# yesint/molar

Hardware: AMD Instinct MI355X
Metric: frames/sec + Matom-pairs/sec, 1M-atom PBC neighbor search + RMSD fit (higher is better)
Workload: dtype f32; 1 GPU; 1M-atom synthetic triclinic box A, per frame: PBC neighbour search rc=1.2 nm (ordered pair list in HBM) + Kabsch RMSD fit/COM/gyration of a 100k-atom selection; natoms=1000000, selection_atoms=100000, frames_per_gpu=1451, parallelism=frames sharded over 1 rank(s), no data-path collective, streams_per_gpu=2, measure_overlapped_with_search=True

## Files before the change

include/molar_hip.h:

```cpp
#ifndef MOLAR_HIP_H
#define MOLAR_HIP_H

#include <stddef.h>
#include <stdint.h>

#ifdef __cplusplus
extern "C" {
#endif

enum {
    MOLAR_HIP_OK = 0,
    MOLAR_HIP_ERR_SIZES = 1,
    MOLAR_HIP_ERR_ZERO_MASS = 2,
    MOLAR_HIP_ERR_SVD = 3,
    MOLAR_HIP_ERR_NO_PBC = 4,
    MOLAR_HIP_ERR_ZERO_LENGTH_VECTOR = 5,
    MOLAR_HIP_ERR_INVERSE_FAILED = 6,
    MOLAR_HIP_ERR_LIPID_TAIL_TOO_SHORT = 7,
    MOLAR_HIP_ERR_LIPID_NORMALS_COUNT = 8,
    MOLAR_HIP_ERR_LIPID_BOND_ORDER_COUNT = 9,
    MOLAR_HIP_ERR_ANGLE_TOO_SMALL = 10,
    MOLAR_HIP_ERR_INVALID_ARGUMENT = 50,
    MOLAR_HIP_ERR_TOO_LARGE = 51,
    MOLAR_HIP_ERR_NO_SEARCH = 52,
// ... 35 lines not shown
int molar_hip_box_from_vectors_angles(float a, float b, float c, float alpha, float beta, float gamma,
                                      molar_hip_box *out);
void molar_hip_box_shortest_vector(const molar_hip_box *box, const float v[3], uint8_t pbc, float out[3]);
void molar_hip_box_lab_extents(const molar_hip_box *box, float out[3]);
void molar_hip_box_extents(const molar_hip_box *box, float out[3]);
void molar_hip_box_to_box_coords(const molar_hip_box *box, const float v[3], float out[3]);
void molar_hip_box_to_lab_coords(const molar_hip_box *box, const float v[3], float out[3]);
int molar_hip_box_is_inside(const molar_hip_box *box, const float p[3]);
void molar_hip_box_wrap_point(const molar_hip_box *box, const float p[3], float out[3]);


enum {
    MOLAR_HIP_SEARCH_SINGLE = 0,
    MOLAR_HIP_SEARCH_DOUBLE = 1,
    MOLAR_HIP_SEARCH_WITHIN = 2,
    MOLAR_HIP_SEARCH_DOUBLE_VDW = 3
};

typedef struct {
    int32_t kind;
    float cutoff;
    const float *xyz1;
    size_t natoms1;
    const uint64_t *idx1;
    size_t n1;
    const float *xyz2;
    size_t natoms2;
    const uint64_t *idx2;
    size_t n2;
    const float *vdw1;
    const float *vdw2;
    int32_t ids_local;
    const float *box9;
    uint8_t pbc;
    const float *lower3;
    const float *upper3;
} molar_hip_search_desc;

int molar_hip_search_count(molar_hip_ctx *ctx, const molar_hip_search_desc *desc, uint64_t *out_count);
int molar_hip_search_fill(molar_hip_ctx *ctx, uint32_t *pairs, float *dist);
int molar_hip_search_fill_usize(molar_hip_ctx *ctx, uint64_t *i, uint64_t *j, float *dist);
int molar_hip_search_fill_ids(molar_hip_ctx *ctx, uint64_t *ids);
int molar_hip_within_count(molar_hip_ctx *ctx, const molar_hip_search_desc *desc, uint64_t *out_count);
int molar_hip_within_fill(molar_hip_ctx *ctx, uint64_t *ids);
int molar_hip_within_hold(molar_hip_ctx *ctx, int on);
int molar_hip_search_connectivity(molar_hip_ctx *ctx, const molar_hip_search_desc *desc, uint64_t *out_rows, uint64_t *out_entries);
int molar_hip_search_connectivity_fill(molar_hip_ctx *ctx, uint64_t *offsets, uint64_t *neigh);
int molar_hip_unwrap_connectivity(molar_hip_ctx *ctx, float *xyz, size_t natoms, const uint64_t *idx, size_t n,
                                  const float *box9, float cutoff, uint8_t pbc_dims, uint64_t *group_offsets,
                                  uint64_t *group_ids, size_t *ngroups);
int molar_hip_search_grid_dims(molar_hip_ctx *ctx, uint64_t dims[3]);
int molar_hip_search_cell_kernels(molar_hip_ctx *ctx, int32_t *lanes, uint64_t occupied_cells[2]);
int molar_hip_search_slot_counts(molar_hip_ctx *ctx, uint64_t *slots, uint64_t *consecutive_slots);
int molar_hip_search_fill_device(molar_hip_ctx *ctx, const uint32_t **d_pairs, const float **d_dist);
int molar_hip_search_resident(molar_hip_ctx *ctx, const molar_hip_search_desc *desc, uint64_t *out_count,
                              const uint32_t **d_pairs, const float **d_dist);
int molar_hip_search_resident_planes(molar_hip_ctx *ctx, int want_dist);
int molar_hip_search_resident_begin(molar_hip_ctx *ctx, const molar_hip_search_desc *desc, int32_t *ticket);
int molar_hip_search_resident_end(molar_hip_ctx *ctx, int32_t ticket, uint64_t *out_count, const uint32_t **d_pairs,
                                  const float **d_dist);
int molar_hip_search_histogram(molar_hip_ctx *ctx, const molar_hip_search_desc *desc, float hmin,
                               float hmax, size_t nbins, uint64_t *bins, uint64_t *out_count);
int molar_hip_search_histogram_frames(molar_hip_ctx *ctx, const molar_hip_search_desc *desc, size_t nframes, size_t xyz1_stride,
                                      size_t xyz2_stride, const float *boxes9, float hmin, float hmax, size_t nbins,
                                      uint64_t *bins);
int molar_hip_histogram_edges(float hmin, float hmax, size_t nbins, float *edges);

typedef struct {
    const uint32_t *group1;
    size_t ngroups1;
    const uint32_t *group2;
    size_t ngroups2;
} molar_hip_contact_groups;

int molar_hip_search_contacts(molar_hip_ctx *ctx, const molar_hip_search_desc *desc, const molar_hip_contact_groups *groups ,
                              uint64_t *deg1, uint64_t *deg2, uint64_t *map, uint64_t *out_count);
int molar_hip_search_contacts_frames(molar_hip_ctx *ctx, const molar_hip_search_desc *desc, const molar_hip_contact_groups *groups,
                                     size_t nframes, size_t xyz1_stride, size_t xyz2_stride, const float *boxes9,
                                     uint64_t *deg1, uint64_t *deg2, uint64_t *map, uint32_t *occupancy);

int molar_hip_search_clusters(molar_hip_ctx *ctx, const molar_hip_search_desc *desc, const molar_hip_contact_groups *groups ,
                              uint32_t *comp_of, uint32_t *sizes, uint64_t *offsets, uint32_t *members, uint32_t *out_ncomponents);
int molar_hip_search_clusters_frames(molar_hip_ctx *ctx, const molar_hip_search_desc *desc, const molar_hip_contact_groups *groups,
                                     size_t nframes, size_t xyz1_stride, const float *boxes9, uint32_t *ncomponents, uint32_t *largest,
                                     uint64_t *size_hist, uint32_t *comp_of_frames);
int molar_hip_search_clusters_counters(molar_hip_ctx *ctx, int32_t enable, uint64_t *out4);

enum {
    MOLAR_HIP_HBOND_DHA_MIN = 0,
    MOLAR_HIP_HBOND_HDA_MAX = 1
};
int molar_hip_hbonds_count(molar_hip_ctx *ctx, const molar_hip_search_desc *desc, const uint64_t *h_offsets, const uint64_t *h_idx,
                           size_t nh, int32_t angle_kind, double angle_deg, double max_ha, uint64_t *out_count);
int molar_hip_hbonds_fill(molar_hip_ctx *ctx, uint32_t *triples, double *dist_da, double *dist_ha, double *angle_deg);
int molar_hip_hbonds_counts(molar_hip_ctx *ctx, const molar_hip_search_desc *desc, const uint64_t *h_offsets, const uint64_t *h_idx,
                            size_t nh, int32_t angle_kind, double angle_deg, double max_ha, const molar_hip_contact_groups *groups,
                            uint64_t *don_count, uint64_t *acc_count, uint64_t *map, uint64_t *out_count);
int molar_hip_hbonds_frames(molar_hip_ctx *ctx, const molar_hip_search_desc *desc, const uint64_t *h_offsets, const uint64_t *h_idx,
                            size_t nh, int32_t angle_kind, double angle_deg, double max_ha, size_t nframes, size_t xyz_stride,
                            const float *boxes9, const molar_hip_contact_groups *groups, uint64_t *per_frame, uint64_t *don_count,
                            uint64_t *acc_count, uint64_t *map, uint64_t *out_total, uint64_t *out_unique);
int molar_hip_hbonds_frames_fill(molar_hip_ctx *ctx, uint64_t *frame_offsets, uint32_t *triples, double *dist_da, double *dist_ha,
                                 double *angle_deg, uint32_t *bond_of_entry, uint32_t *table, uint32_t *occupancy);

int molar_hip_lifetimes_plan(size_t nframes, size_t nrows, size_t ngroups, int want_cont, size_t *workspace_bytes,
                             uint32_t *words_per_row);
// ... 480 lines not shown
```

molar_amd/_lib.py:

```python
from __future__ import annotations

import ctypes as C
import os

HERE = os.path.dirname(os.path.abspath(__file__))
DEFAULT_LIB = os.path.join(HERE, "libmolar_hip.so")

_lib = None


class MolarHipError(RuntimeError):

    def __init__(self, code: int, msg: str):
        super().__init__(f"[molar_hip status {code}] {msg}")
        self.code = code


class Box(C.Structure):
    _fields_ = [("m", C.c_float * 9), ("inv", C.c_float * 9), ("nshift", C.c_int32), ("shifts", C.c_float * 78)]


class SearchDesc(C.Structure):
    _fields_ = [
        ("kind", C.c_int32), ("cutoff", C.c_float),
# ... 49 lines not shown
        ("masses", C.c_void_p), ("ntails", C.c_size_t), ("tail_idx", C.c_void_p), ("tail_offsets", C.c_void_p),
        ("tail_lipid", C.c_void_p), ("tail_bonds", C.c_void_p),
        ("cutoff", C.c_float), ("order_type", C.c_int32), ("max_smooth_iter", C.c_int32), ("unwrap", C.c_int32),
        ("use_global_normal", C.c_int32), ("global_normal", C.c_float * 3),
    ]


MEMBRANE_ARRAYS = ("head", "mid", "tail", "patch_offsets", "patch_ids", "initial_normals", "valid", "smoothed_head", "normals",
                   "quad_coefs", "mean_curv", "gauss_curv", "princ_curvs", "princ_dirs", "area", "nvert", "neib_ids",
                   "voro_vertexes", "fitted_patch_points", "order")


class MembraneView(C.Structure):
    _fields_ = ([("nlipids", C.c_size_t), ("patch_entries", C.c_size_t), ("npairs", C.c_size_t)]
                + [(k, C.c_void_p) for k in MEMBRANE_ARRAYS] + [("norder", C.c_size_t)])


class MembraneOut(C.Structure):
    _fields_ = [(k, C.c_void_p) for k in MEMBRANE_ARRAYS]


_P, _SZ, _F, _I, _U8 = C.c_void_p, C.c_size_t, C.c_float, C.c_int, C.c_uint8
SYMBOLS = {
    "molar_hip_create": (C.c_void_p, [_I]),
    "molar_hip_destroy": (None, [_P]),
    "molar_hip_last_error": (C.c_char_p, []),
    "molar_hip_version": (C.c_char_p, []),
    "molar_hip_device_count": (_I, []),
    "molar_hip_set_stream": (_I, [_P, _P]),
    "molar_hip_synchronize": (_I, [_P]),
    "molar_hip_profile_enable": (_I, [_P, _I]),
    "molar_hip_profile_read": (_I, [_P, _P, _P]),
    "molar_hip_box_from_matrix": (_I, [_P, _P]),
    "molar_hip_box_from_vectors_angles": (_I, [_F, _F, _F, _F, _F, _F, _P]),
    "molar_hip_box_shortest_vector": (None, [_P, _P, _U8, _P]),
    "molar_hip_copy_bandwidth": (_I, [_P, _SZ, _I, _P]),
    "molar_hip_write_bandwidth": (_I, [_P, _SZ, _I, _P]),
    "molar_hip_box_lab_extents": (None, [_P, _P]),
    "molar_hip_box_extents": (None, [_P, _P]),
    "molar_hip_box_to_box_coords": (None, [_P, _P, _P]),
    "molar_hip_box_to_lab_coords": (None, [_P, _P, _P]),
    "molar_hip_box_is_inside": (_I, [_P, _P]),
    "molar_hip_box_wrap_point": (None, [_P, _P, _P]),
    "molar_hip_search_count": (_I, [_P, _P, _P]),
    "molar_hip_search_fill": (_I, [_P, _P, _P]),
    "molar_hip_search_fill_usize": (_I, [_P, _P, _P, _P]),
    "molar_hip_search_fill_ids": (_I, [_P, _P]),
    "molar_hip_within_count": (_I, [_P, _P, _P]),
    "molar_hip_within_fill": (_I, [_P, _P]),
    "molar_hip_within_hold": (_I, [_P, _I]),
    "molar_hip_search_grid_dims": (_I, [_P, _P]),
    "molar_hip_search_cell_kernels": (_I, [_P, _P, _P]),
    "molar_hip_search_slot_counts": (_I, [_P, _P, _P]),
    "molar_hip_search_count_f64": (_I, [_P, _P, _P]),
    "molar_hip_search_fill_f64": (_I, [_P, _P, _P, _P]),
    "molar_hip_search_fill_ids_f64": (_I, [_P, _P]),
    "molar_hip_search_grid_dims_f64": (_I, [_P, _P]),
    "molar_hip_search_histogram_f64": (_I, [_P, _P, C.c_double, C.c_double, _SZ, _P, _P]),
    "molar_hip_search_histogram_frames_f64": (_I, [_P, _P, _SZ, _SZ, _SZ, _P, C.c_double, C.c_double, _SZ, _P]),
    "molar_hip_histogram_edges_f64": (_I, [C.c_double, C.c_double, _SZ, _P]),
    "molar_hip_within_count_f64": (_I, [_P, _P, _P]),
    "molar_hip_within_fill_f64": (_I, [_P, _P]),
    "molar_hip_search_connectivity_f64": (_I, [_P, _P, _P, _P]),
    "molar_hip_unwrap_connectivity_f64": (_I, [_P, _P, _SZ, _P, _SZ, _P, C.c_double, _U8, _P, _P, _P]),
    "molar_hip_search_resident": (_I, [_P, _P, _P, _P, _P]),
    "molar_hip_search_fill_device": (_I, [_P, _P, _P]),
    "molar_hip_search_resident_planes": (_I, [_P, _I]),
    "molar_hip_search_resident_begin": (_I, [_P, _P, _P]),
    "molar_hip_search_resident_end": (_I, [_P, C.c_int32, _P, _P, _P]),
    "molar_hip_search_histogram": (_I, [_P, _P, _F, _F, _SZ, _P, _P]),
    "molar_hip_search_histogram_frames": (_I, [_P, _P, _SZ, _SZ, _SZ, _P, _F, _F, _SZ, _P]),
    "molar_hip_histogram_edges": (_I, [_F, _F, _SZ, _P]),
    "molar_hip_search_contacts": (_I, [_P, _P, _P, _P, _P, _P, _P]),
    "molar_hip_search_contacts_frames": (_I, [_P, _P, _P, _SZ, _SZ, _SZ, _P, _P, _P, _P, _P]),
    "molar_hip_search_clusters": (_I, [_P, _P, _P, _P, _P, _P, _P, _P]),
    "molar_hip_search_clusters_frames": (_I, [_P, _P, _P, _SZ, _SZ, _P, _P, _P, _P, _P]),
    "molar_hip_search_clusters_counters": (_I, [_P, C.c_int32, _P]),
    "molar_hip_min_max": (_I, [_P, _P, _SZ, _P, _SZ, _P, _P]),
    "molar_hip_center_of_geometry": (_I, [_P, _P, _SZ, _P, _SZ, _P]),
    "molar_hip_center_of_mass": (_I, [_P, _P, _SZ, _P, _SZ, _P, _P]),
    "molar_hip_center_of_geometry_pbc": (_I, [_P, _P, _SZ, _P, _SZ, _P, _U8, _P]),
    "molar_hip_center_of_mass_pbc": (_I, [_P, _P, _SZ, _P, _SZ, _P, _P, _U8, _P]),
    "molar_hip_gyration": (_I, [_P, _P, _SZ, _P, _SZ, _P, _P, _P]),
    "molar_hip_inertia": (_I, [_P, _P, _SZ, _P, _SZ, _P, _P, _P, _P, _P]),
    "molar_hip_rmsd": (_I, [_P, _P, _SZ, _P, _SZ, _P, _SZ, _P, _SZ, _P]),
    "molar_hip_rmsd_mw": (_I, [_P, _P, _SZ, _P, _SZ, _P, _P, _SZ, _P, _SZ, _P]),
    "molar_hip_fit_transform": (_I, [_P, _P, _SZ, _P, _SZ, _P, _P, _SZ, _P, _SZ, _P, _I, _P, _P]),
    "molar_hip_xtc_histogram": (_I, [_P, _P, _SZ, _SZ, _P, _SZ, _F, _U8, _F, _F, _SZ, _P, _I]),
    "molar_hip_xtc_histogram_double": (_I, [_P, _P, _SZ, _SZ, _P, _SZ, _P, _SZ, _F, _U8, _F, _F, _SZ, _P, _I]),
    "molar_hip_fit_stream_create": (_I, [_P, _SZ, _P, _SZ, _P, _P, _SZ, _P, _I, _P]),
    "molar_hip_fit_stream_begin": (_I, [_P, _P, _I, _P]),
    "molar_hip_fit_stream_end": (_I, [_P, C.c_int32, _P, _P, _P, _P, _P]),
    "molar_hip_fit_stream_destroy": (None, [_P]),
    "molar_hip_center_of_geometry_f64": (_I, [_P, _P, _SZ, _P, _SZ, _P]),
    "molar_hip_center_of_mass_f64": (_I, [_P, _P, _SZ, _P, _SZ, _P, _P]),
    "molar_hip_gyration_f64": (_I, [_P, _P, _SZ, _P, _SZ, _P, _P]),
    "molar_hip_rmsd_f64": (_I, [_P, _P, _SZ, _P, _SZ, _P, _SZ, _P, _SZ, _P]),
    "molar_hip_rmsd_mw_f64": (_I, [_P, _P, _SZ, _P, _SZ, _P, _P, _SZ, _P, _SZ, _P]),
    "molar_hip_fit_transform_f64": (_I, [_P, _P, _SZ, _P, _SZ, _P, _P, _SZ, _P, _SZ, _P, _I, _P, _P]),
    "molar_hip_apply_transform_f64": (_I, [_P, _P, _SZ, _P, _SZ, _P, _P]),
    "molar_hip_fit_rmsd_batch_f64": (_I, [_P, _P, _SZ, _SZ, _P, _SZ, _P, _P, _SZ, _P, _I, _P, _P, _P, _P, _P]),
    "molar_hip_center_of_geometry_pbc_f64": (_I, [_P, _P, _SZ, _P, _SZ, _P, _U8, _P]),
    "molar_hip_center_of_mass_pbc_f64": (_I, [_P, _P, _SZ, _P, _SZ, _P, _P, _U8, _P]),
    "molar_hip_gyration_pbc_f64": (_I, [_P, _P, _SZ, _P, _SZ, _P, _P, _P]),
    "molar_hip_unwrap_simple_f64": (_I, [_P, _P, _SZ, _P, _SZ, _P, _U8]),
    "molar_hip_inertia_pbc_f64": (_I, [_P, _P, _SZ, _P, _SZ, _P, _P, _P, _P, _P]),
# ... 140 lines not shown
```

molar_amd/api.py:

```python
from __future__ import annotations

import collections
import ctypes as C

import numpy as np

from . import _lib
from ._lib import (MEMBRANE_ARRAYS, Box, ContactGroups, MembraneDesc, MembraneOut, MembraneView, MolarHipError, SearchDesc, SearchDescF64,
                   check)

PBC_FULL = 7
PBC_NONE = 0

SEARCH_SINGLE, SEARCH_DOUBLE, SEARCH_WITHIN, SEARCH_DOUBLE_VDW = 0, 1, 2, 3

ERR_NO_SEARCH = 52
LIFETIME_OUTPUTS = ("inter", "cont", "run_hist", "events", "longest", "present")


def _is_torch(x) -> bool:
    return type(x).__module__.startswith("torch")


def _addr(x):
# ... 202 lines not shown
        d = SearchDesc()
        d.kind = kind
        d.cutoff = float(cutoff) if cutoff is not None else 0.0
        keep = []
        for name, arr in (("xyz1", xyz1), ("idx1", idx1), ("xyz2", xyz2), ("idx2", idx2), ("vdw1", vdw1),
                          ("vdw2", vdw2)):
            a, k = _addr(arr)
            setattr(d, name, a)
            keep.append(k)
        d.natoms1 = 0 if xyz1 is None else xyz1.shape[0] if xyz1.ndim == 2 else xyz1.shape[0] // 3
        d.natoms2 = 0 if xyz2 is None else xyz2.shape[0] if xyz2.ndim == 2 else xyz2.shape[0] // 3
        d.n1 = 0 if idx1 is None else idx1.shape[0]
        d.n2 = 0 if idx2 is None else idx2.shape[0]
        d.ids_local = 1 if ids_local else 0
        if box is not None:
            b9 = box.colmajor9() if isinstance(box, PeriodicBox) else np.ascontiguousarray(
                np.asarray(box, np.float32).reshape(3, 3).T).reshape(9)
            keep.append(b9)
            d.box9 = b9.ctypes.data
        d.pbc = pbc_mask(pbc)
        if lower is not None:
            lo = np.ascontiguousarray(lower, np.float32); up = np.ascontiguousarray(upper, np.float32)
            keep += [lo, up]
            d.lower3 = lo.ctypes.data
            d.upper3 = up.ctypes.data
        return d, keep

    def search_count(self, kind, cutoff, xyz1, idx1=None, xyz2=None, idx2=None, box=None, pbc=0, vdw1=None,
                     vdw2=None, ids_local=False, lower=None, upper=None) -> int:
        d, keep = self._search_desc(kind, cutoff, xyz1, idx1, xyz2, idx2, box, pbc, vdw1, vdw2, ids_local, lower, upper)
        cnt = C.c_uint64(0)
        check(self.lib.molar_hip_search_count(self.ctx, C.byref(d), C.byref(cnt)))
        self._keep = keep
        return int(cnt.value)

    def make_search_desc(self, kind, cutoff, xyz1, **kw):
        return self._search_desc(kind, cutoff, xyz1, **kw)

    def search_resident_desc(self, desc):
        cnt = C.c_uint64(0); p = C.c_void_p(); dd = C.c_void_p()
        check(self.lib.molar_hip_search_resident(self.ctx, C.byref(desc), C.byref(cnt), C.byref(p), C.byref(dd)))
        return int(cnt.value), p.value, dd.value

    def search_cell_kernels(self):
        lanes = C.c_int32(-1)
        occ = (C.c_uint64 * 2)()
        check(self.lib.molar_hip_search_cell_kernels(self.ctx, C.byref(lanes), occ))
        return int(lanes.value), (int(occ[0]), int(occ[1]))

    def search_slot_counts(self):
        slots, rows = C.c_uint64(0), C.c_uint64(0)
        check(self.lib.molar_hip_search_slot_counts(self.ctx, C.byref(slots), C.byref(rows)))
        return int(slots.value), int(rows.value)

    def search_resident_planes(self, want_dist=True):
        check(self.lib.molar_hip_search_resident_planes(self.ctx, 1 if want_dist else 0))

    def search_resident_begin(self, desc):
        t = C.c_int32(-1)
        check(self.lib.molar_hip_search_resident_begin(self.ctx, C.byref(desc), C.byref(t)))
        return int(t.value)

    def search_resident_end(self, ticket):
        cnt = C.c_uint64(0); p = C.c_void_p(); dd = C.c_void_p()
        check(self.lib.molar_hip_search_resident_end(self.ctx, C.c_int32(ticket), C.byref(cnt), C.byref(p), C.byref(dd)))
        return int(cnt.value), p.value, dd.value

    def search_resident(self, kind, cutoff, xyz1, idx1=None, xyz2=None, idx2=None, box=None, pbc=0, vdw1=None,
                        vdw2=None, ids_local=False, lower=None, upper=None):
        d, keep = self._search_desc(kind, cutoff, xyz1, idx1, xyz2, idx2, box, pbc, vdw1, vdw2, ids_local, lower, upper)
        cnt = C.c_uint64(0); p = C.c_void_p(); dd = C.c_void_p()
        check(self.lib.molar_hip_search_resident(self.ctx, C.byref(d), C.byref(cnt), C.byref(p), C.byref(dd)))
        self._keep = keep
        return int(cnt.value), p.value, dd.value

    def search_fill(self, count):
        pairs = np.empty((count, 2), np.uint32)
        dist = np.empty(count, np.float32)
        check(self.lib.molar_hip_search_fill(self.ctx, pairs.ctypes.data, dist.ctypes.data))
        return pairs, dist

    def search_fill_usize(self, count):
        i = np.empty(count, np.uint64); j = np.empty(count, np.uint64); d = np.empty(count, np.float32)
        check(self.lib.molar_hip_search_fill_usize(self.ctx, i.ctypes.data, j.ctypes.data, d.ctypes.data))
        return i, j, d

    def within_set(self, cutoff, xyz1, idx1=None, xyz2=None, idx2=None, box=None, pbc=0, ids_local=False, lower=None,
                   upper=None, device_out=None):
        d, keep = self._search_desc(SEARCH_WITHIN, cutoff, xyz1, idx1, xyz2, idx2, box, pbc, None, None, ids_local, lower, upper)
        cnt = C.c_uint64(0)
        check(self.lib.molar_hip_within_count(self.ctx, C.byref(d), C.byref(cnt)))
        self._keep = keep
        n = int(cnt.value)
        if device_out is not None:
            out = device_out(n)
            if n:
                check(self.lib.molar_hip_within_fill(self.ctx, out.data_ptr()))
            return out
        ids = np.empty(n, np.uint64)
        if n:
            check(self.lib.molar_hip_within_fill(self.ctx, ids.ctypes.data))
        return ids

    def search_connectivity(self, cutoff, xyz, idx=None, box=None, pbc=0, ids_local=True):
        d, keep = self._search_desc(SEARCH_SINGLE, cutoff, xyz, idx, None, None, box, pbc, None, None, ids_local, None, None)
        rows, ent = C.c_uint64(0), C.c_uint64(0)
# ... 2913 lines not shown
```

molar_amd/csrc/api.hip:

```cpp
#include "boxmath.hpp"
#include <algorithm>

#include "common.hpp"
#include "hoststream.hpp"
#include <cstdlib>

using namespace mh;

typedef float v4f_copy __attribute__((ext_vector_type(4)));
__global__ __launch_bounds__(256) void k_copy_f4(const float4 *__restrict__ src, float4 *__restrict__ dst, size_t n) {
    for (size_t i = (size_t)blockIdx.x * 256u + threadIdx.x; i < n; i += (size_t)gridDim.x * 256u) dst[i] = src[i];
}
template <bool NT>
__global__ __launch_bounds__(256) void k_copy_f4x4(const v4f_copy *__restrict__ src, v4f_copy *__restrict__ dst, size_t n) {
    for (size_t i = (size_t)blockIdx.x * 1024u + threadIdx.x; i < n; i += (size_t)gridDim.x * 1024u) {
        v4f_copy v0, v1, v2, v3;
        if (NT) {
            v0 = __builtin_nontemporal_load(src + i);
            v1 = __builtin_nontemporal_load(src + i + 256);
            v2 = __builtin_nontemporal_load(src + i + 512);
            v3 = __builtin_nontemporal_load(src + i + 768);
            __builtin_nontemporal_store(v0, dst + i);
            __builtin_nontemporal_store(v1, dst + i + 256);
            __builtin_nontemporal_store(v2, dst + i + 512);
// ... 77 lines not shown

const char *molar_hip_last_error(void) { return last_error().c_str(); }

const char *molar_hip_version(void) { return "molar_hip 0.2 (gfx950)"; }

int molar_hip_device_count(void) {
    int n = 0;
    if (hipGetDeviceCount(&n) != hipSuccess) {
        (void)hipGetLastError();
        return 0;
    }
    return n;
}

molar_hip_ctx *molar_hip_create(int device) {
    int n = 0;
    hipError_t e = hipGetDeviceCount(&n);
    if (e != hipSuccess || n == 0) {
        (void)hipGetLastError();
        fail(MOLAR_HIP_ERR_HIP, "molar_hip_create: no HIP device visible (%s)",
             e == hipSuccess ? "device count is 0" : hipGetErrorString(e));
        return nullptr;
    }
    if (device < 0 || device >= n) {
        fail(MOLAR_HIP_ERR_INVALID_ARGUMENT, "molar_hip_create: device %d out of range [0,%d)", device, n);
        return nullptr;
    }
    if ((e = hipSetDevice(device)) != hipSuccess) {
        fail(MOLAR_HIP_ERR_HIP, "hipSetDevice(%d): %s", device, hipGetErrorString(e));
        return nullptr;
    }
    hipDeviceProp_t prop;
    if ((e = hipGetDeviceProperties(&prop, device)) != hipSuccess) {
        fail(MOLAR_HIP_ERR_HIP, "hipGetDeviceProperties: %s", hipGetErrorString(e));
        return nullptr;
    }
    auto *c = new molar_hip_ctx();
    c->device = device;
    c->num_cus = prop.multiProcessorCount > 0 ? prop.multiProcessorCount : 256;
    if ((e = hipStreamCreateWithFlags(&c->stream, hipStreamNonBlocking)) != hipSuccess) {
        fail(MOLAR_HIP_ERR_HIP, "hipStreamCreate: %s", hipGetErrorString(e));
        delete c;
        return nullptr;
    }
    c->own_stream = true;
#ifdef MOLAR_HIP_AB_KNOBS
    c->env_no_side = std::getenv("MOLAR_HIP_NO_SIDE_STREAM") != nullptr;
    c->env_no_mfma = std::getenv("MOLAR_HIP_NO_MFMA_COUNT") != nullptr;
    c->env_no_mfma_wrapped = std::getenv("MOLAR_HIP_NO_MFMA_WRAPPED") != nullptr;
    c->env_no_tile_sum = std::getenv("MOLAR_HIP_NO_TILE_SUM") != nullptr;
    c->env_host_grid_wait = std::getenv("MOLAR_HIP_HOST_GRID_WAIT") != nullptr;
    c->env_no_bin_tile = std::getenv("MOLAR_HIP_NO_BIN_TILE") != nullptr;
#endif
#ifdef MOLAR_HIP_DEBUG_KNOBS
    if (const char *dbg = std::getenv("MOLAR_HIP_DEBUG_SKIP")) c->env_debug_skip = (uint32_t)std::atoi(dbg);
    if (const char *dbg = std::getenv("MOLAR_HIP_DEBUG_LAUNCH")) c->env_debug_launch = (uint32_t)std::atoi(dbg);
#endif
    if (ensure_pinned(c, 1 << 16) || alloc_search_sizes(c)) {
        if (c->h_pinned) (void)hipHostFree(c->h_pinned);
        (void)hipStreamDestroy(c->stream);
        delete c;
        return nullptr;
    }
    return c;
}

void molar_hip_destroy(molar_hip_ctx *c) {
    if (!c) return;
    (void)hipSetDevice(c->device);
    (void)hipStreamSynchronize(c->stream);
    if (c->side_stream) (void)hipStreamSynchronize(c->side_stream);
    if (c->aux) molar_hip_destroy(c->aux);
    mh::contacts_release(c);
    if (c->hb_pin) (void)hipHostFree(c->hb_pin);
    for (auto e : c->hb_pin_ev)
        if (e) (void)hipEventDestroy(e);
    for (auto &s : c->spans) {
        (void)hipEventDestroy(s.a);
        (void)hipEventDestroy(s.b);
    }
    for (auto e : c->event_pool) (void)hipEventDestroy(e);
    if (c->h_pinned) (void)hipHostFree(c->h_pinned);
    mh::ring_release(c);
    mh::search64_release(c);
    mh::sasa_release(c);
    mh::rmsd_matrix_release(c);
    mh::fluct_release(c);
    mh::msd_release(c);
    mh::density_release(c);
    mh::intcoord_release(c);
    mh::tcf_release(c);
    mh::sfactor_release(c);
    mh::mindist_release(c);
    mh::hbonds_release(c);
    mh::lifetimes_release(c);
    mh::within_release(c);
    mh::connectivity_release(c);
    if (c->h_sizes) (void)hipHostFree(c->h_sizes);
    for (auto &t : c->tickets)
        if (t.done) (void)hipEventDestroy(t.done);
    if (c->grid_done) (void)hipEventDestroy(c->grid_done);
    for (auto e : c->gen_free)
        if (e) (void)hipEventDestroy(e);
    if (c->side_stream) (void)hipStreamDestroy(c->side_stream);
    if (c->own_stream) (void)hipStreamDestroy(c->stream);
    delete c;
// ... 127 lines not shown
```

molar_amd/csrc/common.hpp:

```cpp
#pragma once

#include <hip/hip_runtime.h>

#include <cstdarg>
#include <cstddef>
#include <cstdint>
#include <cstdio>
#include <cstring>
#include <string>
#include <utility>
#include <vector>

#include "../../include/molar_hip.h"

namespace mh {


inline std::string &last_error() {
    static thread_local std::string e;
    return e;
}

inline int fail(int code, const char *fmt, ...) {
    char buf[512];
// ... 151 lines not shown
struct molar_hip_sfactor_state;
struct molar_hip_mindist_state;
struct molar_hip_hbonds_state;
struct molar_hip_lifetimes_state;
struct molar_hip_within_state;
struct molar_hip_connectivity_state;
struct molar_hip_contacts_state;

#ifndef MH_HIST_BATCH
#define MH_HIST_BATCH 16
#endif

struct molar_hip_ctx {
    int device = 0;
    hipStream_t stream = nullptr;
    bool own_stream = false;
    int num_cus = 256;

    void *h_pinned = nullptr;
    size_t h_pinned_cap = 0;
    molar_hip_search64_state *s64 = nullptr;
    molar_hip_sasa_state *sasa = nullptr;
    molar_hip_rmsd_matrix_state *rmsdm = nullptr;
    molar_hip_fluct_state *fluct = nullptr;
    molar_hip_msd_state *msd = nullptr;
    molar_hip_density_state *density = nullptr;
    molar_hip_intcoord_state *intcoord = nullptr;
    molar_hip_tcf_state *tcf = nullptr;
    molar_hip_sfactor_state *sfactor = nullptr;
    molar_hip_mindist_state *mindist = nullptr;
    molar_hip_hbonds_state *hbonds = nullptr;
    molar_hip_lifetimes_state *lifetimes = nullptr;
    molar_hip_within_state *within = nullptr;
    molar_hip_connectivity_state *conn = nullptr;
    molar_hip_contacts_state *contacts = nullptr;
    void *ring[8] = {nullptr, nullptr, nullptr, nullptr, nullptr, nullptr, nullptr, nullptr};
    hipEvent_t ring_ev[8] = {nullptr, nullptr, nullptr, nullptr, nullptr, nullptr, nullptr, nullptr};

    bool have_search = false;
    mh::SearchShape cur;
    uint64_t total = 0;
    mh::GridSet set_store[2][2];
    molar_hip_ctx() { cur.set = set_store[0]; }
    hipStream_t side_stream = nullptr;
    hipEvent_t grid_done = nullptr;
    bool env_no_side = false;
    bool env_no_mfma = false;
    bool env_no_mfma_wrapped = false;
    bool env_host_grid_wait = false;
    bool env_no_tile_sum = false;
    uint32_t env_debug_skip = 0;
    uint32_t env_debug_launch = 0, dbg_launches = 0;
    hipEvent_t gen_free[2] = {nullptr, nullptr};
    bool env_no_bin_tile = false;
    int hist_gen = 0;
    mh::DevBuf scan_tmp_side;
    mh::DevBuf params;
    mh::DevBuf task_desc;
    mh::DevBuf task_nb;
    mh::DevBuf slot_desc;
    mh::DevBuf slot_cnt;
    mh::DevBuf slot_base;
    mh::DevBuf tile_sum;
    bool params_fresh = false;
    unsigned long long params_fresh_cap = 0;
    mh::DevBuf scan_tmp;
    mh::DevBuf sort_tmp, sort_tmp_side;
    mh::DevBuf scan_state;
    mh::DevBuf fplan_tiles;
    mh::DevBuf slot_stat;
    bool slot_stat_valid = false;
    bool plan_live = false;
    mh::DevBuf out_pairs_set[2];
    mh::DevBuf out_dist_set[2];
    mh::DevBuf &out_pairs = out_pairs_set[0];
    mh::DevBuf &out_dist = out_dist_set[0];
    struct Ticket {
        bool pending = false, degenerate = false;
        unsigned long long cap0 = 0, maskcap0 = 0, serial = 0, launched = 0, ntasks = 0;
        int kind = -1;
        unsigned long long occ_key = 0;
        hipEvent_t done = nullptr;
        molar_hip_search_desc desc{};
    } tickets[2];
    int next_ticket = 0;
    bool resident_no_dist = false;
    unsigned long long search_serial = 0;
    unsigned long long trim_real = 0, trim_ntasks = 0;
    int trim_kind = -1;
    static constexpr int SIZES_SYNC = 2, SIZES_ENTRIES = 3;
    mh::SearchSizes *h_sizes = nullptr, *d_sizes = nullptr;
    unsigned long long occ_key = 0;
    uint32_t occ_cells[2] = {0, 0};
    bool occ_valid = false;
    mh::DevBuf out_ids;
    mh::DevBuf wide_i, wide_j;
    mh::DevBuf hist;
    mh::DevBuf dbg;
    mh::DevBuf hist_queue;
    mh::DevBuf slot_desc_rest;
    unsigned long long hist_frames = 0;
    mh::GridSet hb_sets[2][MH_HIST_BATCH][2];
    bool hb_zeroed[2][MH_HIST_BATCH][2] = {};
    uint32_t hb_zeroed_cells[2][MH_HIST_BATCH][2] = {};
    mh::DevBuf hb_lean[2], hb_rest[2];
    mh::DevBuf hb_blocks[2];
    void *hb_pin = nullptr;
    hipEvent_t hb_pin_ev[4] = {nullptr, nullptr, nullptr, nullptr};
    bool hb_pin_used[4] = {false, false, false, false};
    unsigned hb_pin_next = 0;
    mh::DevBuf hist_edges;
    float edges_min = 0.f, edges_max = 0.f;
    size_t edges_nbins = 0;
    bool within_hold = false;
    mh::HeldGrid held;
    mh::DevBuf task_mu;
    mh::DevBuf task_moff;
    mh::DevBuf maskbuf;
    uint64_t mask_units = 0;

    molar_hip_ctx *aux = nullptr;
    mh::DevBuf xh_win[2], xh_bins;

    bool profiling = false;
    bool profile_frames = false;
    struct Span { int cls; hipEvent_t a, b; };
    std::vector<Span> spans;
    std::vector<hipEvent_t> event_pool;

    mh::DevBuf fit_redo;
    mh::DevBuf m_xyz1, m_xyz2, m_idx1, m_idx2, m_mass1, m_mass2, m_partials, m_results, m_out;
};

namespace mh {

void search64_release(molar_hip_ctx *c);
void sasa_release(molar_hip_ctx *c);
void rmsd_matrix_release(molar_hip_ctx *c);
void fluct_release(molar_hip_ctx *c);
void msd_release(molar_hip_ctx *c);
void density_release(molar_hip_ctx *c);
void intcoord_release(molar_hip_ctx *c);
void tcf_release(molar_hip_ctx *c);
void sfactor_release(molar_hip_ctx *c);
void mindist_release(molar_hip_ctx *c);
void hbonds_release(molar_hip_ctx *c);
void lifetimes_release(molar_hip_ctx *c);
void within_release(molar_hip_ctx *c);
void connectivity_release(molar_hip_ctx *c);
void contacts_release(molar_hip_ctx *c);


template <class State>
State &state_of(State *&slot) {
    if (!slot) slot = new State;
    return *slot;
}

template <class State>
void release_state(State *&slot) {
    delete slot;
    slot = nullptr;
}

struct HbondsBlockView {
    const uint64_t *frame_offsets;
    size_t nframes;
    const uint32_t *bond_of_entry;
    size_t rows, entries;
    uint64_t serial;
};
// ... 88 lines not shown
```

molar_amd/csrc/pair_kernels.hpp:

```cpp
#pragma once

#include "boxmath.hpp"
#include "common.hpp"

namespace mh {
namespace pairk {

enum { MODE_COUNT = 0, MODE_FILL = 1, MODE_HIST = 2 };

#ifndef MH_COUNT_WPE
#define MH_COUNT_WPE 6
#endif
#ifndef MH_FILL_WPE
#define MH_FILL_WPE 8
#endif
#ifndef MH_WPB
#define MH_WPB 1
#endif
constexpr int waves_per_block(int mode) { return mode == MODE_HIST ? 4 : MH_WPB; }
constexpr int KREG = 8;
constexpr int FIFO_CAP = 128;
constexpr int LIVE_GROUPS = KREG;
constexpr uint32_t SLOT_LIVE = 0x400u;
#ifndef MOLAR_HIP_NO_WIDE_FLUSH
// ... 25 lines not shown
__device__ __forceinline__ void gstore_u32(uint32_t *p, size_t i, uint32_t v) {
    ((__attribute__((address_space(1))) uint32_t *)p)[i] = v;
}
__device__ __forceinline__ float uniform_f32(float v) { return __uint_as_float(__builtin_amdgcn_readfirstlane(__float_as_uint(v))); }
__device__ __forceinline__ float4 lload4(const float4 *p, uint32_t i) {
    const v4f_t v = ((const __attribute__((address_space(3))) v4f_t *)p)[i];
    return make_float4(v.x, v.y, v.z, v.w);
}

struct SearchParams {
    const float4 *sa;
    const float4 *sb;
    const uint32_t *csa;
    const uint32_t *csb;
    const float *vdwa;
    const float *vdwb;
    const float4 *aabb_b;
    const float4 *perm_b;
    const float4 *chunk_aabb_b;
    const uint4 *h16_b;
    const float4 *cell_org_b;
    uint32_t mfma_count;
    const struct TaskDesc *task_desc;
    uint32_t *maskbuf;
    const unsigned long long *task_moff;
    unsigned long long mask_cap_units;
    unsigned long long out_cap;
    uint32_t dx, dy, dz;
    uint32_t pbc;
    uint32_t use_box;
    uint32_t nblocks;
    uint32_t wrap_kind;
    uint32_t prune_wrapped;
    float prune_limit2;
    uint32_t approx_wrapped;
    float band_lo, band_hi;
    uint32_t hist_nbins;
    float hist_min, hist_max;
    unsigned long long *hist_bins;
    unsigned long long *hist_total;
    const float *hist_edges;
    float hist_scale;
    uint32_t hist_lean;
    const uint32_t *hist_nslots;
#ifdef MOLAR_HIP_DEBUG_KNOBS
    uint32_t debug_skip;
    unsigned long long *dbg;
#endif
    float cutoff2;
    uint64_t ntasks;
    molar_hip_box box;
    alignas(16) float shifts4[96];
    uint32_t hist_big;
};

struct TaskDesc {
    uint32_t a0, n1, b0, n2, cb, flags, pad0, pad1;
};

struct SlotDesc {
    uint32_t a0, n1, b0, n2;
    uint32_t cb, flags, i0, frame;
    unsigned long long moff, pad1;
};
static_assert(sizeof(SlotDesc) == 48, "SlotDesc is read with three 16-byte loads");

struct Task {
    uint32_t a0, n1, b0, n2;
    uint32_t rps;
    uint32_t cb;
    uint32_t ca;
    uint32_t wrap_b;
    uint32_t wrap;
    bool tri;
    bool valid;
};

struct SlotTask : Task {
    bool live = false;
    uint32_t lrow = 0;
};

__device__ __forceinline__ uint32_t slot_row(const SlotTask &T, uint32_t i0, uint32_t lane) { return T.live ? T.lrow : i0 + lane; }

template <int KIND, bool UNIFORM>
__device__ __forceinline__ Task decode_task(const SearchParams &P, uint64_t t) {
    Task T;
    T.valid = false;
    T.tri = false;
    T.a0 = T.b0 = T.n1 = T.n2 = 0;
    T.cb = 0;
    T.ca = 0;
    T.wrap_b = 0;
    T.rps = 64u;
    T.wrap = 0;
    uint32_t half = 0;
    uint64_t e = t;
    if (KIND != MOLAR_HIP_SEARCH_SINGLE) {
        half = (uint32_t)(t & 1ull);
        e = t >> 1;
    }
    const uint32_t m = (uint32_t)(e % 14ull);
    const uint64_t cidx = e / 14ull;
    const uint32_t z = (uint32_t)(cidx % P.dz);
    const uint64_t r = cidx / P.dz;
    const uint32_t y = (uint32_t)(r % P.dy);
    const uint32_t x = (uint32_t)(r / P.dy);
    const uint32_t dims[3] = {P.dx, P.dy, P.dz};
    uint32_t c[2][3] = {{x + MASKS[m][0], y + MASKS[m][1], z + MASKS[m][2]},
                        {x + MASKS[m][3], y + MASKS[m][4], z + MASKS[m][5]}};
    uint32_t wrap = 0, wrap_c2 = 0;
    for (int i = 0; i < 2; ++i)
        for (int d = 0; d < 3; ++d)
            if (c[i][d] == dims[d]) {
                if ((P.pbc >> d) & 1u) {
                    c[i][d] = 0;
                    wrap |= 1u << d;
                    if (i == 1) wrap_c2 |= 1u << d;
                } else {
                    return T;
                }
            }
    const uint32_t i1 = c[0][0] + c[0][1] * P.dx + c[0][2] * P.dx * P.dy;
    const uint32_t i2 = c[1][0] + c[1][1] * P.dx + c[1][2] * P.dx * P.dy;
    uint32_t ca = i1, cb = i2;
    if (KIND == MOLAR_HIP_SEARCH_SINGLE) {
        T.tri = (i1 == i2);
    } else if (half) {
        ca = i2;
        cb = i1;
    }
    T.a0 = P.csa[ca];
    T.n1 = P.csa[ca + 1] - T.a0;
    T.b0 = P.csb[cb];
// ... 518 lines not shown
    const uint32_t rank = TRI ? lane : __builtin_amdgcn_mbcnt_hi((uint32_t)(live >> 32), __builtin_amdgcn_mbcnt_lo((uint32_t)live, 0u));
    u4_t bq[MFMA_TILES];
#pragma unroll
    for (int t = 0; t < MFMA_TILES; ++t) {
        const uint32_t col = (uint32_t)t * 32u + cl;
        if (32u * (uint32_t)(t + 1) <= T.n2) {
            bq[t] = ((const glb_u4 *)P.h16_b)[T.b0 + col];
        } else {
            bq[t] = u4_t{0u, 0u, 0u, 0x00007BFFu};
            if (col < T.n2) bq[t] = ((const glb_u4 *)P.h16_b)[T.b0 + col];
        }
    }
    if (TRI || need) la[rank] = a;
    const float r0 = a.x - org.x, r1 = a.y - org.y, r2 = a.z - org.z;
    float ra2 = need ? (r0 * r0 + r1 * r1) + r2 * r2 : 0.0f;
    const bool fin = ra2 == ra2;
    for (int off = 32; off > 0; off >>= 1) ra2 = fmaxf(ra2, __shfl_xor(ra2, off, 64));
    const float R = 1.0001f * __builtin_sqrtf(ra2) + org.w;
    const float E = uniform_f32(mfma_error_bound(R, cutoff2));
    if (__builtin_amdgcn_ballot_w64(!fin) != 0ull || !mfma_bound_usable(R, E, cutoff2)) {
        done = false;
        return 0u;
    }
    {
        u4_t k0 = {0u, 0u, 0u, 0x00007BFFu}, k1 = {0u, 0u, 0u, 0x3C003C00u};
        if (!TRI) {
            ((lds_u4 *)lh)[2u * lane] = k0;
            ((lds_u4 *)lh)[2u * lane + 1u] = k1;
            __builtin_amdgcn_wave_barrier();
        }
        if (need) {
            const _Float16 h0 = (_Float16)r0, h1 = (_Float16)r1, h2 = (_Float16)r2;
            const _Float16 l0 = (_Float16)(r0 - (float)h0), l1 = (_Float16)(r1 - (float)h1), l2 = (_Float16)(r2 - (float)h2);
            const float e0 = (float)h0 + (float)l0, e1 = (float)h1 + (float)l1, e2 = (float)h2 + (float)l2;
            const float na = ((e0 * e0 + e1 * e1) + e2 * e2) - cutoff2;
            const _Float16 nh = (_Float16)na, nl = (_Float16)(na - (float)nh);
            const _Float16 m2 = (_Float16)-2.0f;
            const _Float16 g0 = m2 * h0, g1 = m2 * h1, g2 = m2 * h2, s0 = m2 * l0, s1 = m2 * l1, s2 = m2 * l2;
            k0 = u4_t{pack_h2(g0, g1), pack_h2(g2, g0), pack_h2(g1, g2), pack_h2(nh, nl)};
            k1 = u4_t{pack_h2(s0, s1), pack_h2(s2, s0), pack_h2(s1, s2), 0x3C003C00u};
        }
        if (TRI || need) {
            ((lds_u4 *)lh)[2u * rank] = k0;
            ((lds_u4 *)lh)[2u * rank + 1u] = k1;
        }
    }
    __builtin_amdgcn_wave_barrier();
    const u4_t a0q = ((const lds_u4 *)lh)[2u * cl + kh], a1q = ((const lds_u4 *)lh)[2u * (32u + cl) + kh];
    const v8h_t A0 = __builtin_bit_cast(v8h_t, a0q), A1 = __builtin_bit_cast(v8h_t, a1q);
    __builtin_amdgcn_wave_barrier();
    lds_u32 *todo = (lds_u32 *)lh;
    uint32_t ntodo = 0;
    uint32_t cnt = 0;
#pragma unroll
    for (int t = 0; t < MFMA_TILES; ++t) {
        if ((uint32_t)t < nct) {
            u4_t bt = bq[t];
            if (kh == 0u) bt.w = 0x3C003C00u;
            const v8h_t B = __builtin_bit_cast(v8h_t, bt);
#pragma unroll
            for (int rt = 0; rt < 2; ++rt) {
                bool diag = false;
                if (32u * (uint32_t)rt >= nlive) continue;
                if (TRI) {
                    const uint32_t row0 = i0 + 32u * (uint32_t)rt;
                    if (32u * (uint32_t)t + 31u <= row0) continue;
                    diag = 32u * (uint32_t)t <= row0 + 31u;
                }
                v16f_t acc = {0.f, 0.f, 0.f, 0.f, 0.f, 0.f, 0.f, 0.f, 0.f, 0.f, 0.f, 0.f, 0.f, 0.f, 0.f, 0.f};
                acc = __builtin_amdgcn_mfma_f32_32x32x16_f16(rt == 0 ? A0 : A1, B, acc, 0, 0, 0);
                if (TRI && diag) {
                    const int tv = (int)(32u * (uint32_t)t + cl) - (int)(i0 + 32u * (uint32_t)rt + 4u * kh);
#pragma unroll
                    for (int i = 0; i < 16; ++i) acc[i] = (tv > 8 * (i / 4) + (i % 4)) ? acc[i] : 1.0e30f;
                }
                uint32_t h = 0u;
                float m = INFINITY;
#pragma unroll
                for (int i = 0; i < 16; ++i) {
                    h = __builtin_amdgcn_alignbit(h, __float_as_uint(acc[i]), 31);
                    m = __builtin_fminf(m, __builtin_fabsf(acc[i]));
                }
                if (__builtin_amdgcn_ballot_w64(m < E) == 0ull) {
                    cnt += (uint32_t)__popc(h);
                } else {
                    if (lane == 0) todo[ntodo] = (uint32_t)(2 * t + rt);
                    ++ntodo;
                }
            }
        }
    }
    if (ntodo) {
        __builtin_amdgcn_wave_barrier();
        for (uint32_t q = 0; q < ntodo; ++q) {
            const uint32_t id = __builtin_amdgcn_readfirstlane(todo[q]);
            const uint32_t ct = id >> 1, rt = id & 1u;
            const uint32_t col = ct * 32u + cl;
            float4 b = make_float4(3.0e38f, 3.0e38f, 3.0e38f, 0.f);
            if (col < T.n2) b = gload4(P.sb, T.b0 + col);
            for (uint32_t r = 0; r < 16u; ++r) {
                const uint32_t row = 32u * rt + 16u * kh + r;
                const float4 p = lload4(la, row);
                const float dx = b.x - p.x, dy = b.y - p.y, dz = b.z - p.z;
                const float d2 = (dx * dx + dy * dy) + dz * dz;
                cnt += (row < nlive && (!TRI || col > i0 + row) && d2 <= cutoff2) ? 1u : 0u;
            }
        }
    }
    for (int off = 32; off > 0; off >>= 1) cnt += __shfl_xor(cnt, off, 64);
    return cnt;
}

template <int KIND>
__device__ __forceinline__ bool run_count_mfma_wrapped(const SearchParams &P, const SlotTask &T, uint32_t i0, float4 *la, uint4 *lh,
                                                       uint32_t lane, uint32_t *mwords, uint32_t &count_out) {
    typedef uint32_t u4_t __attribute__((ext_vector_type(4)));
    typedef __attribute__((address_space(3))) u4_t lds_u4;
    typedef __attribute__((address_space(3))) uint32_t lds_u32;
    typedef __attribute__((address_space(1))) u4_t glb_u4;
    const float cutoff2 = P.cutoff2;
    const uint32_t rows = __builtin_amdgcn_readfirstlane(T.n1 - i0 < 64u ? T.n1 - i0 : 64u);
    const uint32_t kh = lane >> 5, cl = lane & 31u;
    const uint32_t nct = (T.n2 + 31u) >> 5, nch = (T.n2 + 63u) >> 6;
    float Sx = 0.f, Sy = 0.f, Sz = 0.f;
    for (int d = 0; d < 3; ++d) {
        if (!((T.wrap >> d) & 1u)) continue;
        const float sgn = ((T.wrap_b >> d) & 1u) ? 1.0f : -1.0f;
        Sx += sgn * P.box.m[3 * d];
        Sy += sgn * P.box.m[3 * d + 1];
        Sz += sgn * P.box.m[3 * d + 2];
    }
    float4 a = make_float4(0.f, 0.f, 0.f, 0.f);
    if (lane < rows) a = gload4(P.sa, T.a0 + slot_row(T, i0, lane));
    const float4 org = gload4(P.cell_org_b, T.cb);
    bool need = lane < rows;
    if (!T.live) {
        const float4 blo = gload4(P.aabb_b, 2 * T.cb), bhi = gload4(P.aabb_b, 2 * T.cb + 1);
        need = need && !(aabb_d2(a.x - Sx, a.y - Sy, a.z - Sz, blo.x, blo.y, blo.z, bhi.x, bhi.y, bhi.z) > P.prune_limit2);
    }
    const unsigned long long live = __builtin_amdgcn_ballot_w64(need);
    const uint32_t nlive = (uint32_t)__popcll(live);
    if (nlive == 0u) {
        count_out = 0u;
// ... 94 lines not shown
                const uint32_t hy = (uint32_t)(2 * k + 1) < nct ? block(2 * k + 1, rt) : 0u;
                const uint32_t got = (uint32_t)__shfl_xor((int)(kh ? hx : hy), 32, 64);
                const uint32_t half0 = kh ? got : hx, half1 = kh ? hy : got;
                const uint32_t word = (spread(half0) << 4) | spread(half1);
                cnt += (uint32_t)__popc(word);
                gstore_u32(mwords, ((uint32_t)rt * nch + (uint32_t)k) * 64u + lane, word);
            }
        }
    }
    if (ntodo > TODO_CAP) return false;
    if (ntodo) {
        asm volatile("s_waitcnt vmcnt(0)" ::: "memory");
        __builtin_amdgcn_wave_barrier();
        for (uint32_t q0 = 0; q0 < ntodo; q0 += 64u) {
            bool hx = false;
            uint32_t rl = 0u, col = 0u;
            if (q0 + lane < ntodo) {
                const uint32_t e = todo[q0 + lane];
                rl = e >> 16;
                col = e & 0xFFFFu;
                if (rl < nlive && col < T.n2) {
                    const float4 b = gload4(P.sb, T.b0 + col);
                    const float4 p = lload4(la, rl);
                    hx = wrapped_d2_exact(P, T.wrap, b.x - p.x, b.y - p.y, b.z - p.z) <= cutoff2;
                }
            }
            if (hx) atomicOr(mwords + ((rl >> 5) * nch + (col >> 6)) * 64u + (col & 63u), 0x80000000u >> (rl & 31u));
            const unsigned long long mx = __builtin_amdgcn_ballot_w64(hx);
            if (lane == 0) cnt += (uint32_t)__popcll(mx);
        }
    }
    for (int off = 32; off > 0; off >>= 1) cnt += __shfl_xor(cnt, off, 64);
    count_out = cnt;
    return true;
}

template <int KIND, bool FILL, bool WRAPPED, int NCH, bool TRI, bool MASKED>
__device__ __forceinline__ uint32_t run_fast(const SearchParams &P, const SlotTask &T, uint32_t i0, Fifo &F, float4 *la,
                                             uint32_t lane, uint32_t *mwords) {
    static_assert(!(WRAPPED && TRI), "a triangular (same-cell) entry never wraps on the fast path");
    if constexpr (!FILL && !WRAPPED && MASKED_COUNT_SORTED) return run_count_sorted<KIND, NCH, TRI>(P, T, i0, la, lane);
    const bool approx = WRAPPED && P.approx_wrapped != 0u && !(P.box.nshift != 0 && T.wrap == MOLAR_HIP_PBC_FULL);
    float Sx = 0.f, Sy = 0.f, Sz = 0.f;
    if (WRAPPED && approx) {
        for (int d = 0; d < 3; ++d) {
            if (!((T.wrap >> d) & 1u)) continue;
            const float sgn = ((T.wrap_b >> d) & 1u) ? 1.0f : -1.0f;
            Sx += sgn * P.box.m[3 * d];
            Sy += sgn * P.box.m[3 * d + 1];
            Sz += sgn * P.box.m[3 * d + 2];
        }
    }
    constexpr bool REPLAY = FILL && MASKED;
    float bx[NCH], by[NCH], bz[NCH];
    uint32_t bid[NCH];
    if (!REPLAY) {
#pragma unroll
        for (int k = 0; k < NCH; ++k) {
            const uint32_t jj = (uint32_t)k * 64u + lane;
            float4 q = make_float4(3.0e38f, 3.0e38f, 3.0e38f, 0.f);
            if (jj < T.n2) {
                q = gload4(P.sb, T.b0 + jj);
                if (WRAPPED) { q.x += Sx; q.y += Sy; q.z += Sz; }
            }
            bx[k] = q.x; by[k] = q.y; bz[k] = q.z; bid[k] = __float_as_uint(q.w);
        }
    }
    const float cutoff2 = P.cutoff2;
    const float band_lo = P.band_lo, band_hi = P.band_hi;
    const uint32_t rows = __builtin_amdgcn_readfirstlane(T.n1 - i0 < T.rps ? T.n1 - i0 : T.rps);
    unsigned long long live;
    {
        float4 a = make_float4(0.f, 0.f, 0.f, 0.f);
        if (lane < rows) a = gload4(P.sa, T.a0 + slot_row(T, i0, lane));
        la[lane] = a;
        float4 lo = make_float4(0.f, 0.f, 0.f, 0.f), hi = lo;
        if (!T.live) {
            lo = gload4(P.aabb_b, 2 * T.cb);
            hi = gload4(P.aabb_b, 2 * T.cb + 1);
        }
        bool need = true;
        if (TRI || T.live) {
        } else if (!WRAPPED) {
            need = !(aabb_d2(a.x, a.y, a.z, lo.x, lo.y, lo.z, hi.x, hi.y, hi.z) > cutoff2);
        } else if (approx) {
            need = !(aabb_d2(a.x - Sx, a.y - Sy, a.z - Sz, lo.x, lo.y, lo.z, hi.x, hi.y, hi.z) > P.prune_limit2);
        }
        live = __builtin_amdgcn_ballot_w64(lane < rows && need);
    }
    __builtin_amdgcn_wave_barrier();
    uint32_t total = 0;

    if (REPLAY) {
        if (!mwords) return 0u;
        F.recompute = WRAPPED ? 1u : 2u;
        F.la = la;
        F.wrap = T.wrap;
        F.fq = F.fq_store;
        float4 q[NCH];
#pragma unroll
        for (int k = 0; k < NCH; ++k) {
            const uint32_t jj = (uint32_t)k * 64u + lane;
            q[k] = make_float4(0.f, 0.f, 0.f, 0.f);
            if (jj < T.n2) q[k] = gload4(P.sb, T.b0 + jj);
        }
        uint32_t w[NCH];
// ... 24 lines not shown
                    total += cnt;
                    if (F.tail - F.head >= 64u) fifo_drain<KIND>(P, F, lane);
                }
            }
        }
        if (F.tail != F.head) {
            __builtin_amdgcn_wave_barrier();
            fifo_flush<KIND>(P, F, F.tail - F.head, lane);
        }
        F.recompute = 0u;
        F.fq = nullptr;
        return total;
    }

#ifdef MOLAR_HIP_WIDE_FLUSH
    constexpr bool WIDE = FILL && !WRAPPED && KIND != MOLAR_HIP_SEARCH_WITHIN;
#else
    constexpr bool WIDE = false;
#endif
    if (FILL) {
        F.recompute = (WRAPPED && approx) ? 1u : 0u;
        F.la = la;
        F.wrap = T.wrap;
        if (WIDE && !F.hist) F.quota = 128u - ((uint32_t)F.base & 127u);
    }
    uint32_t acc = 0;
    uint32_t acc_hi = 0;
    uint32_t hw[NCH];
    uint32_t su = 0, mu = 0;
    uint32_t nrow = 0;
    if (MASKED) {
#pragma unroll
        for (int k = 0; k < NCH; ++k) hw[k] = 0u;
    }
    auto store_group = [&](uint32_t g, uint32_t n) {
#pragma unroll
        for (int k = 0; k < NCH; ++k) {
            acc += (uint32_t)__popc(hw[k]);
            if (mwords) gstore_u32(mwords, (g * NCH + k) * 64u + lane, hw[k] << (32u - n));
            hw[k] = 0u;
        }
    };
    auto exact_d2 = [&](const float4 &p, uint32_t jj) -> float {
        float4 q = make_float4(3.0e38f, 3.0e38f, 3.0e38f, 0.f);
        if (jj < T.n2) q = gload4(P.sb, T.b0 + jj);
        return wrapped_d2_exact(P, T.wrap, q.x - p.x, q.y - p.y, q.z - p.z);
    };
    while (live) {
        const uint32_t r = (uint32_t)__builtin_ctzll(live);
        live &= ~(1ull << r);
        const float4 p = lload4(la, r);
        const uint32_t id_i = __float_as_uint(p.w);
        const uint32_t i = i0 + r;
#pragma unroll
        for (int k = 0; k < NCH; ++k) {
            if (TRI && (uint32_t)k * 64u + 63u <= i) {
                if (MASKED && !FILL) hw[k] += hw[k];
                continue;
            }
            const uint32_t jj = (uint32_t)k * 64u + lane;
            const float dx = bx[k] - p.x, dy = by[k] - p.y, dz = bz[k] - p.z;
            float d2 = (dx * dx + dy * dy) + dz * dz;
            if (WRAPPED && !approx) d2 = wrapped_d2_exact<FILL && !MASKED>(P, T.wrap, dx, dy, dz);
            if (TRI && (uint32_t)k * 64u <= i) d2 = (jj > i) ? d2 : INFINITY;
            if (!FILL) {
                if (MASKED) {
                    if (WRAPPED && approx) {
                        unsigned long long scr;
                        asm volatile("v_cmp_gt_f32 vcc, %4, %3\n\t"
                                     "v_addc_co_u32 %0, %2, %0, %0, vcc\n\t"
                                     "v_addc_co_u32 %1, %2, %1, %1, vcc"
                                     : "+v"(hw[k]), "+v"(su), "=&s"(scr) : "v"(d2), "s"(band_lo) : "vcc");
                        asm volatile("v_cmp_ge_f32 vcc, %2, %1\n\tv_addc_co_u32 %0, vcc, %0, %0, vcc" : "+v"(mu) : "v"(d2), "s"(band_hi) : "vcc");
                    } else {
                        asm volatile("v_cmp_ge_f32 vcc, %2, %1\n\tv_addc_co_u32 %0, vcc, %0, %0, vcc" : "+v"(hw[k]) : "v"(d2), "s"(cutoff2) : "vcc");
                    }
                } else if (WRAPPED && approx) {
                    asm volatile("v_cmp_gt_f32 vcc, %2, %1\n\tv_addc_co_u32 %0, vcc, 0, %0, vcc" : "+v"(acc) : "v"(d2), "s"(band_lo) : "vcc");
                    asm volatile("v_cmp_ge_f32 vcc, %2, %1\n\tv_addc_co_u32 %0, vcc, 0, %0, vcc" : "+v"(acc_hi) : "v"(d2), "s"(band_hi) : "vcc");
                } else {
                    asm volatile("v_cmp_ge_f32 vcc, %2, %1\n\tv_addc_co_u32 %0, vcc, 0, %0, vcc" : "+v"(acc) : "v"(d2), "s"(cutoff2) : "vcc");
                }
            } else {
                bool hit;
                uint32_t third = __float_as_uint(d2);
                if (WRAPPED && approx) {
                    const bool sure = d2 < band_lo, maybe = d2 <= band_hi;
                    hit = sure;
                    if (__builtin_amdgcn_ballot_w64(maybe && !sure)) hit = sure || (maybe && exact_d2(p, jj) <= cutoff2);
                    third = (r << 26) | (T.b0 + jj);
                } else {
                    hit = d2 <= cutoff2;
                }
                const unsigned long long mask = __builtin_amdgcn_ballot_w64(hit);
                if (mask) {
                    const uint32_t cnt = (uint32_t)__popcll(mask);
                    if (hit) {
                        const uint32_t rank = __builtin_amdgcn_mbcnt_hi((uint32_t)(mask >> 32), __builtin_amdgcn_mbcnt_lo((uint32_t)mask, 0u));
                        const uint32_t off = ((rank + F.tail) << 2) & (((WIDE ? FIFO_WIDE : FIFO_CAP) - 1u) << 2);
                        typedef __attribute__((address_space(3))) uint32_t lds_u32;
                        *(lds_u32 *)((__attribute__((address_space(3))) char *)F.fi + off) = id_i;
                        *(lds_u32 *)((__attribute__((address_space(3))) char *)F.fj + off) = bid[k];
                        *(lds_u32 *)((__attribute__((address_space(3))) char *)F.fd + off) = third;
                    }
                    F.tail += cnt;
                    total += cnt;
                    if (WIDE) {
                        if (F.tail - F.head >= 128u) fifo_drain_wide<KIND>(P, F, lane);
// ... 52 lines not shown
template <int KIND, bool FILL, int WK, bool MASKED, int KMAX = KREG>
__device__ __forceinline__ uint32_t run_task_nch(const SearchParams &P, const SlotTask &T, uint32_t i0, Fifo &F, float4 *la,
                                                 uint32_t lane, uint32_t *mwords) {
    const uint32_t nchunks = (T.n2 + 63u) >> 6;
    if constexpr (KMAX > KMAX_WIDE) {
        if ((KIND == MOLAR_HIP_SEARCH_SINGLE || KIND == MOLAR_HIP_SEARCH_DOUBLE) && nchunks > (uint32_t)KREG && nchunks <= (uint32_t)KMAX) {
            constexpr bool WR = WK != WK_NONE;
            const bool tri = KIND == MOLAR_HIP_SEARCH_SINGLE && WK == WK_NONE && T.tri;
            if (!T.tri || tri) {
#define MH_HUGE_CASE(N)                                                                                              \
    if (nchunks <= (uint32_t)(N)) {                                                                                  \
        if (tri) {                                                                                                   \
            if constexpr (KIND == MOLAR_HIP_SEARCH_SINGLE && WK == WK_NONE)                                          \
                return run_fast<KIND, FILL, false, N, true, false>(P, T, i0, F, la, lane, nullptr);                  \
        }                                                                                                            \
        return run_fast<KIND, FILL, WR, N, false, false>(P, T, i0, F, la, lane, nullptr);                            \
    }
                MH_HUGE_CASE(16) MH_HUGE_CASE(20) MH_HUGE_CASE(24) MH_HUGE_CASE(28) MH_HUGE_CASE(32)
#undef MH_HUGE_CASE
            }
        }
    } else if constexpr (KMAX > KREG) {
        if ((KIND == MOLAR_HIP_SEARCH_SINGLE || KIND == MOLAR_HIP_SEARCH_DOUBLE) && nchunks > (uint32_t)KREG && nchunks <= (uint32_t)KMAX) {
            constexpr bool WR = WK != WK_NONE;
            const bool tri = KIND == MOLAR_HIP_SEARCH_SINGLE && WK == WK_NONE && T.tri;
            if (!T.tri || tri) {
#define MH_WIDE_CASE(N)                                                                                              \
    case N:                                                                                                          \
        if (tri) {                                                                                                   \
            if constexpr (KIND == MOLAR_HIP_SEARCH_SINGLE && WK == WK_NONE)                                          \
                return run_fast<KIND, FILL, false, N, true, false>(P, T, i0, F, la, lane, nullptr);                  \
        }                                                                                                            \
        return run_fast<KIND, FILL, WR, N, false, false>(P, T, i0, F, la, lane, nullptr);
                switch (nchunks) {
                    MH_WIDE_CASE(9) MH_WIDE_CASE(10) MH_WIDE_CASE(11) MH_WIDE_CASE(12)
                    MH_WIDE_CASE(13) MH_WIDE_CASE(14) MH_WIDE_CASE(15)
                    default: break;
                }
                if (tri) {
                    if constexpr (KIND == MOLAR_HIP_SEARCH_SINGLE && WK == WK_NONE)
                        return run_fast<KIND, FILL, false, 16, true, false>(P, T, i0, F, la, lane, nullptr);
                }
                return run_fast<KIND, FILL, WR, 16, false, false>(P, T, i0, F, la, lane, nullptr);
#undef MH_WIDE_CASE
            }
        }
    }
    if constexpr (!FILL && WK == WK_NONE && (KIND == MOLAR_HIP_SEARCH_SINGLE || KIND == MOLAR_HIP_SEARCH_DOUBLE)) {
        if ((P.mfma_count & 1u) && F.lh && T.n2 <= 32u * (uint32_t)MFMA_TILES) {
            bool done = true;
            const uint32_t cm = (KIND == MOLAR_HIP_SEARCH_SINGLE && T.tri) ? run_count_mfma<KIND, true>(P, T, i0, la, F.lh, lane, done)
                                                                          : run_count_mfma<KIND, false>(P, T, i0, la, F.lh, lane, done);
            if (done) return cm;
        }
    }
    if constexpr (!FILL && MASKED && WK != WK_NONE && (KIND == MOLAR_HIP_SEARCH_SINGLE || KIND == MOLAR_HIP_SEARCH_DOUBLE)) {
        if ((P.mfma_count & 2u) && F.lh && mwords && !T.tri && T.rps == 64u && T.n2 <= 32u * (uint32_t)MFMA_TILES && P.approx_wrapped != 0u &&
            !(P.box.nshift != 0 && T.wrap == MOLAR_HIP_PBC_FULL)) {
            uint32_t cw = 0u;
            if (run_count_mfma_wrapped<KIND>(P, T, i0, la, F.lh, lane, mwords, cw)) return cw;
            __builtin_amdgcn_wave_barrier();
        }
    }
    if ((KIND == MOLAR_HIP_SEARCH_SINGLE || KIND == MOLAR_HIP_SEARCH_DOUBLE) && !T.tri && nchunks <= (uint32_t)KREG) {
        constexpr bool WR = WK != WK_NONE;
        switch (nchunks) {
            case 1: return run_fast<KIND, FILL, WR, 1, false, MASKED && WR>(P, T, i0, F, la, lane, mwords);
            case 2: return run_fast<KIND, FILL, WR, 2, false, MASKED && WR>(P, T, i0, F, la, lane, mwords);
            case 3: return run_fast<KIND, FILL, WR, 3, false, MASKED && WR>(P, T, i0, F, la, lane, mwords);
            case 4: return run_fast<KIND, FILL, WR, 4, false, MASKED && WR>(P, T, i0, F, la, lane, mwords);
            case 5: return run_fast<KIND, FILL, WR, 5, false, MASKED && WR>(P, T, i0, F, la, lane, mwords);
            case 6: return run_fast<KIND, FILL, WR, 6, false, MASKED && WR>(P, T, i0, F, la, lane, mwords);
            case 7: return run_fast<KIND, FILL, WR, 7, false, MASKED && WR>(P, T, i0, F, la, lane, mwords);
            default: return run_fast<KIND, FILL, WR, 8, false, MASKED && WR>(P, T, i0, F, la, lane, mwords);
        }
    }
    if (KIND == MOLAR_HIP_SEARCH_SINGLE && WK == WK_NONE && T.tri && nchunks <= (uint32_t)KREG) {
        switch (nchunks) {
            case 1: return run_fast<KIND, FILL, false, 1, true, false>(P, T, i0, F, la, lane, mwords);
            case 2: return run_fast<KIND, FILL, false, 2, true, false>(P, T, i0, F, la, lane, mwords);
            case 3: return run_fast<KIND, FILL, false, 3, true, false>(P, T, i0, F, la, lane, mwords);
            case 4: return run_fast<KIND, FILL, false, 4, true, false>(P, T, i0, F, la, lane, mwords);
            case 5: return run_fast<KIND, FILL, false, 5, true, false>(P, T, i0, F, la, lane, mwords);
            case 6: return run_fast<KIND, FILL, false, 6, true, false>(P, T, i0, F, la, lane, mwords);
            case 7: return run_fast<KIND, FILL, false, 7, true, false>(P, T, i0, F, la, lane, mwords);
            default: return run_fast<KIND, FILL, false, 8, true, false>(P, T, i0, F, la, lane, mwords);
        }
    }
    if (nchunks > (uint32_t)KREG) {
        if (KIND == MOLAR_HIP_SEARCH_SINGLE && T.tri) return run_task<KIND, FILL, WK, true, 0, false, FILL && !MASKED>(P, T, i0, F, lane);
        return run_task<KIND, FILL, WK, false, 0, false, FILL && !MASKED>(P, T, i0, F, lane);
    }
    if (KIND == MOLAR_HIP_SEARCH_SINGLE && T.tri) return run_task<KIND, FILL, WK, true, KREG, true, FILL && !MASKED>(P, T, i0, F, lane);
    return run_task<KIND, FILL, WK, false, KREG, true, FILL && !MASKED>(P, T, i0, F, lane);
}

template <int KIND>
__global__ void __launch_bounds__(256) plan_kernel(SearchParams P, uint32_t *__restrict__ task_nb,
                                                   TaskDesc *__restrict__ task_desc, uint32_t *__restrict__ task_mu,
                                                   uint32_t fast_kind, uint32_t *__restrict__ slot_cnt, uint64_t nslot_cnt,
                                                   unsigned long long *__restrict__ scan_state, uint64_t nstate,
                                                   SearchParams *__restrict__ params_dst) {
    const uint64_t t = (uint64_t)blockIdx.x * blockDim.x + threadIdx.x;
    if (t < nslot_cnt) slot_cnt[t] = 0u;
    if (t < nstate) scan_state[t] = 0ull;
    if (params_dst && blockIdx.x == 0) {
// ... 109 lines not shown
            const uint32_t x = w & 7u, q = w >> 3;
            const uint32_t full = (nslots / (8u * XCD_RUN)) * (8u * XCD_RUN);
            if (w < full) wr = ((q / XCD_RUN) * 8u + x) * XCD_RUN + (q % XCD_RUN);
        }
        const uint32_t slot = nslots - 1u - wr;
        SlotTask T;
        uint32_t i0;
        unsigned long long moff;
        uint32_t frame = 0u;
        {
            const uint4 lo = reinterpret_cast<const uint4 *>(slot_desc + slot)[0];
            const uint4 hi = reinterpret_cast<const uint4 *>(slot_desc + slot)[1];
            const uint2 mo = reinterpret_cast<const uint2 *>(slot_desc + slot)[4];
            const uint32_t fl = __builtin_amdgcn_readfirstlane(hi.y);
            if (!(fl & 0x200u)) return;
            if (MODE == MODE_HIST) frame = __builtin_amdgcn_readfirstlane(hi.w);
            T.a0 = __builtin_amdgcn_readfirstlane(lo.x);
            T.n1 = __builtin_amdgcn_readfirstlane(lo.y);
            T.b0 = __builtin_amdgcn_readfirstlane(lo.z);
            T.n2 = __builtin_amdgcn_readfirstlane(lo.w);
            T.cb = __builtin_amdgcn_readfirstlane(hi.x);
            i0 = __builtin_amdgcn_readfirstlane(hi.z);
            moff = ((unsigned long long)__builtin_amdgcn_readfirstlane(mo.y) << 32) | __builtin_amdgcn_readfirstlane(mo.x);
            T.wrap = fl & 7u;
            T.tri = (fl & 0x100u) != 0u;
            T.valid = true;
            T.wrap_b = (fl >> 12) & 7u;
            T.rps = fl >> 16;
            if constexpr (LIVE_SLOTS) {
                if (fl & SLOT_LIVE) {
                    typedef __attribute__((address_space(1))) unsigned long long glb_u64;
                    const uint2 mp = reinterpret_cast<const uint2 *>(slot_desc + slot)[5];
                    const glb_u64 *mk = (const glb_u64 *)(((unsigned long long)(uint32_t)__builtin_amdgcn_readfirstlane(mp.y) << 32) |
                                                          (unsigned long long)(uint32_t)__builtin_amdgcn_readfirstlane(mp.x));
                    unsigned long long mw = 0ull;
                    if (lane < (uint32_t)LIVE_GROUPS) mw = mk[lane];
                    uint32_t *scr = lds[wave][0];
                    uint32_t before = 0u;
#pragma unroll
                    for (int g = 0; g < LIVE_GROUPS; ++g) {
                        const uint32_t wlo = __builtin_amdgcn_readlane((uint32_t)mw, g), whi = __builtin_amdgcn_readlane((uint32_t)(mw >> 32), g);
                        const uint32_t n = (uint32_t)__popc(wlo) + (uint32_t)__popc(whi);
                        if (n != 0u && before + n > i0 && before < i0 + 64u) {
                            const uint32_t rank = before + __builtin_amdgcn_mbcnt_hi(whi, __builtin_amdgcn_mbcnt_lo(wlo, 0u)) - i0;
                            const bool bit = (((lane < 32u ? wlo : whi) >> (lane & 31u)) & 1u) != 0u;
                            if (bit && rank < 64u) scr[rank] = 64u * (uint32_t)g + lane;
                        }
                        before += n;
                    }
                    __builtin_amdgcn_wave_barrier();
                    T.lrow = scr[lane];
                    __builtin_amdgcn_wave_barrier();
                    T.live = true;
                    T.n1 = before;
                }
            }
        }
        const SearchParams &P = MODE == MODE_HIST ? Pp[frame] : P0;
        Fifo F;
        F.fi = lds[wave][0];
        F.fj = lds[wave][1];
        F.fd = lds[wave][2];
        F.head = F.tail = 0;
        F.quota = 64u;
        F.has_pairs = out_pairs != nullptr;
        F.has_dist = out_dist != nullptr;
        F.pairs = nullptr;
        F.dist = nullptr;
        F.ids = nullptr;
        F.base = 0;
        F.room = 0xFFFFFFFFu;
        F.hist = hist ? lds_hist : nullptr;
        F.recompute = 0u;
        F.la = lds_a[wave];
        F.fq = nullptr;
        F.fq_store = MODE == MODE_FILL ? reinterpret_cast<float4 *>(lds[wave][0]) : nullptr;
        F.lh = MODE == MODE_COUNT ? lds_h[wave] : nullptr;
        F.wrap = 0;
        F.hmin = P.hist_min;
        F.hmax = P.hist_max;
        F.hn = (float)P.hist_nbins;
        if (FILL && !hist) {
            F.base = slot_base[slot];
            F.quota = 64u - ((uint32_t)F.base & 63u);
            const unsigned long long end = slot_base[slot + 1];
            if (end == F.base || end > P.out_cap) return;
            F.room = end - F.base < 0xFFFFFFFFull ? (uint32_t)(end - F.base) : 0xFFFFFFFFu;
            if (out_pairs) F.pairs = out_pairs + F.base + lane;
            if (out_dist) F.dist = out_dist + F.base + lane;
            if (out_ids) F.ids = out_ids + F.base + lane;
        }
        uint32_t total = 0;
        const uint32_t wk = (P.use_box && T.wrap != 0) ? P.wrap_kind : (uint32_t)WK_NONE;
        if (hist && P.hist_lean && !P.hist_nslots && hist_lean_slot<KIND>(P, (T.tri ? 0x100u : 0u) | T.wrap, T.n2)) return;
#ifdef MOLAR_HIP_DEBUG_KNOBS
        if (P.debug_skip) {
            const uint32_t kind_bit = T.tri ? 4u : (wk != WK_NONE ? (T.rps == 8u ? 8u : 2u) : 1u);
            if (P.debug_skip & kind_bit) return;
        }
#endif
        constexpr bool MASKED = MODE != MODE_HIST;
        uint32_t *mwords = nullptr;
        if (MASKED) {
            const uint32_t nch = (T.n2 + 63u) >> 6;
            if (moff + 2u * nch <= P.mask_cap_units) mwords = P.maskbuf + moff * 64u;
        }
// ... 90 lines not shown
```

molar_amd/csrc/search.hip:

```cpp
#include <cstdlib>

#include "boxmath.hpp"
#include "common.hpp"
#include "csr_kernels.hpp"
#include "hoststream.hpp"
#include <algorithm>

#include "pair_kernels.hpp"
#include "search_core.hpp"
#include "search_shape.hpp"
#include "stages.hpp"

namespace mh {
void launch_pair_small(int mode, int lanes_per_slot, hipStream_t stream, const pairk::SearchParams *dP, const pairk::SlotDesc *slot_desc,
                       uint32_t nslots, uint32_t *slot_cnt, const unsigned long long *slot_base, uint2 *pairs, float *dist);
}
using namespace mh;
using namespace mh::pairk;

namespace {

constexpr uint32_t DROPPED = 0xFFFFFFFFu;


// ... 1010 lines not shown
    }
    if ((threadIdx.x & 63) == 0) {
        for (int d = 0; d < 3; ++d) {
            if (lo[d] != INFINITY) atomicMin(&mm[d], f2ord(lo[d]));
            if (hi[d] != -INFINITY) atomicMax(&mm[3 + d], f2ord(hi[d]));
        }
    }
}

__global__ void __launch_bounds__(256) fmax_kernel(const float *__restrict__ v1, uint32_t n1, const float *__restrict__ v2, uint32_t n2,
                                                   uint32_t *__restrict__ out) {
    const float *v = blockIdx.y ? v2 : v1;
    const uint32_t n = blockIdx.y ? n2 : n1;
    float m = -INFINITY;
    bool any = false;
    for (uint32_t k = blockIdx.x * 256u + threadIdx.x; k < n; k += gridDim.x * 256u) {
        const float x = v[k];
        if (x == x) {
            m = fmaxf(m, x);
            any = true;
        }
    }
    for (int off = 32; off > 0; off >>= 1) m = fmaxf(m, __shfl_xor(m, off, 64));
    const bool wave_any = __ballot(any) != 0ull;
    __shared__ float wm[4];
    __shared__ uint32_t wa[4];
    if ((threadIdx.x & 63) == 0) {
        wm[threadIdx.x >> 6] = m;
        wa[threadIdx.x >> 6] = wave_any ? 1u : 0u;
    }
    __syncthreads();
    if (threadIdx.x == 0 && (wa[0] | wa[1] | wa[2] | wa[3])) {
        float r = -INFINITY;
        for (int w = 0; w < 4; ++w)
            if (wa[w]) r = fmaxf(r, wm[w]);
        atomicMax(out + blockIdx.y, f2ord(r));
    }
}

__global__ void __launch_bounds__(256) widen_pairs_kernel(const uint2 *__restrict__ pairs, uint64_t n,
                                                          unsigned long long *__restrict__ oi,
                                                          unsigned long long *__restrict__ oj) {
    for (uint64_t k = (uint64_t)blockIdx.x * 256u + threadIdx.x; k < n; k += (uint64_t)gridDim.x * 256u) {
        const uint2 p = pairs[k];
        if (oi) oi[k] = p.x;
        if (oj) oj[k] = p.y;
    }
}

__global__ void __launch_bounds__(256) widen_ids_kernel(const uint32_t *__restrict__ ids, uint64_t n,
                                                        unsigned long long *__restrict__ out) {
    for (uint64_t k = (uint64_t)blockIdx.x * 256u + threadIdx.x; k < n; k += (uint64_t)gridDim.x * 256u)
        out[k] = ids[k];
}

__global__ void upload_params_kernel(SearchParams P, SearchParams *dst) {
    const uint32_t *src = (const uint32_t *)__builtin_amdgcn_kernarg_segment_ptr();
    uint32_t *d = (uint32_t *)dst;
    for (uint32_t t = threadIdx.x; t < (uint32_t)(sizeof(SearchParams) / 4u); t += blockDim.x) d[t] = src[t];
}


static void occ_latch(molar_hip_ctx *c) {
    const bool known = c->occ_valid && c->occ_key == occ_key_of(c->cur);
    c->cur.occ_use[0] = known ? c->occ_cells[0] : 0u;
    c->cur.occ_use[1] = known ? c->occ_cells[1] : 0u;
}
static SearchSizes *sizes_dev_of(molar_hip_ctx *c, int i) { return c->d_sizes ? c->d_sizes + i : nullptr; }
static void occ_note(molar_hip_ctx *c, unsigned long long key, const SearchSizes &sizes) {
    if (!key || !(uint32_t)sizes.occupied) return;
    c->occ_key = key;
    c->occ_cells[0] = (uint32_t)sizes.occupied;
    c->occ_cells[1] = (uint32_t)(sizes.occupied >> 32);
    c->occ_valid = true;
}


static int ensure_side_stream(molar_hip_ctx *c) {
    if (c->side_stream) return 0;
    int lo = 0, hi = 0;
    MH_HIP(hipDeviceGetStreamPriorityRange(&lo, &hi));
    MH_HIP(hipStreamCreateWithPriority(&c->side_stream, hipStreamNonBlocking, hi));
    MH_HIP(hipEventCreateWithFlags(&c->grid_done, hipEventDisableTiming));
    return 0;
}

static BinParams grid_bin_params(const SearchShape &shape, const GridSet &S, bool drop_nonfinite) {
    BinParams P{};
    P.xyz = S.d_xyz;
    P.idx = S.d_idx;
    P.n = S.n;
    P.dx = shape.dims[0];
    P.dy = shape.dims[1];
    P.dz = shape.dims[2];
    P.pbc = shape.pbc;
    P.use_box = shape.use_box ? 1u : 0u;
    P.drop_nonfinite = drop_nonfinite ? 1u : 0u;
    for (int d = 0; d < 3; ++d) {
        P.lower[d] = shape.lower[d];
        P.upper[d] = shape.upper[d];
    }
    P.box = shape.box;
    return P;
}

static uint32_t grid_pad_shift(uint32_t n, uint32_t ncells) { return (n && ncells <= (1u << 19) && (uint64_t)n >= 8ull * ncells) ? 5u : 0u; }
// ... 64 lines not shown
        const int want_order = (fixed_cutoff_kind(cur.kind) && (call.hist_plan || small_cell_lanes(cur) == 0)) ? 1 : 0;
        if (!want_order && !by_sort && (uint64_t)S.n < 16ull * ncells)
            hipLaunchKernelGGL(place_small_kernel, dim3((unsigned)(((uint64_t)ncells * 16u + bs - 1u) / bs)), dim3(bs), 0, lane.stream, P, ncells,
                               ids_local, S.cell_count.as<uint32_t>(), S.tmp_key.as<uint32_t>(), S.d_vdw, S.sorted.as<float4>(),
                               S.d_vdw ? S.sorted_vdw.as<float>() : nullptr, S.aabb.as<float4>(), S.cell_org.as<float4>(),
                               S.cell_count.as<uint32_t>() + ncells + 1);
        else
        hipLaunchKernelGGL(place_order_kernel, dim3(ncells), dim3(64), 0, lane.stream, P, ncells, ids_local,
                           S.cell_count.as<uint32_t>(), S.tmp_key.as<uint32_t>(), S.d_vdw, S.sorted.as<float4>(),
                           S.d_vdw ? S.sorted_vdw.as<float>() : nullptr, S.aabb.as<float4>(), S.perm.as<float4>(),
                           S.chunk_aabb.as<float4>(), S.h16.as<uint4>(), S.cell_org.as<float4>(), want_order, by_sort ? 1 : 0,
                           S.cell_count.as<uint32_t>() + ncells + 1);
        MH_HIP(hipGetLastError());
    }
    return 0;
}

int stage_set(molar_hip_ctx *c, GridSet &S, const float *xyz, size_t natoms, const uint64_t *idx, size_t n,
              const float *vdw, bool want_vdw) {
    if (!xyz) return fail(MOLAR_HIP_ERR_INVALID_ARGUMENT, "search: xyz pointer is null");
    const size_t nsel = idx ? n : natoms;
    if (nsel >= 0x7FFFFFFFull || natoms >= 0xFFFFFFFFull)
        return fail(MOLAR_HIP_ERR_TOO_LARGE, "search: %zu atoms exceed the 2^31 limit of the 32-bit device ids", nsel);
    S.n = (uint32_t)nsel;
    MH_TRY(to_device(c, xyz, natoms * 3, S.xyz_stage, &S.d_xyz));
    MH_TRY(to_device(c, idx, idx ? n : 0, S.idx_stage, &S.d_idx));
    S.d_vdw = nullptr;
    if (want_vdw) {
        if (!vdw) return fail(MOLAR_HIP_ERR_INVALID_ARGUMENT, "vdw search: radii pointer is null");
        MH_TRY(to_device(c, vdw, nsel, S.vdw_stage, &S.d_vdw));
    }
    return 0;
}

SearchParams make_params(const molar_hip_ctx *c, const SearchShape &shape) {
    SearchParams P{};
    const GridSet &A = shape.set[0], &B = shape.kind != MOLAR_HIP_SEARCH_SINGLE ? shape.set[1] : shape.set[0];
    P.sa = A.sorted.as<float4>();
    P.csa = A.cell_count.as<uint32_t>();
    P.sb = B.sorted.as<float4>();
    P.csb = B.cell_count.as<uint32_t>();
    P.vdwa = A.sorted_vdw.as<float>();
    P.vdwb = shape.set[1].sorted_vdw.as<float>();
    P.aabb_b = B.aabb.as<float4>();
    P.perm_b = B.perm.as<float4>();
    P.chunk_aabb_b = B.chunk_aabb.as<float4>();
    P.h16_b = B.h16.as<uint4>();
    P.cell_org_b = B.cell_org.as<float4>();
    P.mfma_count = c->env_no_mfma ? 0u : (c->env_no_mfma_wrapped ? 1u : 3u);
    P.task_desc = c->task_desc.as<TaskDesc>();
    P.maskbuf = c->maskbuf.as<uint32_t>();
    P.task_moff = c->task_moff.as<unsigned long long>();
    P.mask_cap_units = c->maskbuf.cap / 256u;
    P.out_cap = ~0ull;
    P.dx = shape.dims[0];
    P.dy = shape.dims[1];
    P.dz = shape.dims[2];
    P.pbc = shape.use_box ? shape.pbc : 0u;
    P.use_box = shape.use_box ? 1u : 0u;
    P.cutoff2 = shape.cutoff * shape.cutoff;
    P.ntasks = shape.ntasks;
    P.nblocks = (uint32_t)shape.nslots_bound;
    P.box = shape.box;
    for (int k = 0; k < 96; ++k) P.shifts4[k] = (shape.use_box && k < 3 * shape.box.nshift) ? shape.box.shifts[k] : 0.0f;
    P.hist_nbins = 0u;
    P.hist_min = P.hist_max = 0.f;
    P.hist_bins = nullptr;
    P.hist_total = nullptr;
    P.hist_nslots = nullptr;
    const WrapPolicy W = wrapped_pair_policy(shape);
    P.wrap_kind = W.wrap_kind;
    P.prune_wrapped = W.prune_wrapped;
    P.approx_wrapped = W.approx_wrapped;
    P.band_lo = W.band_lo;
    P.band_hi = W.band_hi;
    P.prune_limit2 = W.prune_limit2;
#ifdef MOLAR_HIP_DEBUG_KNOBS
    P.debug_skip = c->env_debug_skip;
    P.dbg = nullptr;
#endif
    return P;
}

struct PairOut {
    uint2 *pairs = nullptr;
    float *dist = nullptr;
    uint32_t *ids = nullptr;
};
struct HistTarget {
    uint32_t nbins = 0;
    float min = 0.f, max = 0.f;
    unsigned long long *bins = nullptr;
    unsigned long long *total = nullptr;
};

template <bool FILL>
int launch_pairs(molar_hip_ctx *c, const SearchCall &call, const PairOut &out, const HistTarget &hist = HistTarget{},
                 bool params_resident = false) {
    if (FILL && (((uintptr_t)out.pairs & 15u) || ((uintptr_t)out.dist & 7u)))
        return fail(MOLAR_HIP_ERR_INVALID_ARGUMENT, "search fill: device outputs must be aligned to 16 bytes (pairs) and 8 bytes (distances)");
    Prof prof(c, FILL ? 3 : 1);
    const SearchShape &cur = c->cur;
    SearchParams P = make_params(c, cur);
    if (P.nblocks == 0) return 0;
    P.out_cap = call.out_cap;
    P.hist_nbins = hist.nbins;
// ... 213 lines not shown
            *degenerate = true;
            return 0;
        }
        float m1, m2;
        MH_TRY(device_fmax2(c, cur.set[0].d_vdw, cur.set[0].n, cur.set[1].d_vdw, cur.set[1].n, &m1, &m2));
        cutoff = (m1 + m2) + F32_EPS;
    }
    if (!(cutoff > 0.0f)) return fail(MOLAR_HIP_ERR_INVALID_ARGUMENT, "search: cutoff must be positive (got %g)", (double)cutoff);
    cur.cutoff = cutoff;

    float ext[3];
    if (cur.use_box) {
        molar_hip_box_lab_extents(&cur.box, ext);
    } else {
        if (q->kind == MOLAR_HIP_SEARCH_WITHIN) {
            if (!q->lower3 || !q->upper3)
                return fail(MOLAR_HIP_ERR_INVALID_ARGUMENT, "non-periodic within search needs lower3/upper3");
            for (int d = 0; d < 3; ++d) {
                cur.lower[d] = q->lower3[d];
                cur.upper[d] = q->upper3[d];
            }
        } else {
            MH_TRY(c->hist.reserve(64));
            uint32_t *d_mm = c->hist.as<uint32_t>();
            uint32_t seed[6];
            for (int d = 0; d < 6; ++d) seed[d] = f2ord_host(0.0f);
            MH_HIP(hipMemcpyAsync(d_mm, seed, sizeof seed, hipMemcpyHostToDevice, c->stream));
            MH_TRY(bbox_accumulate(c, d_mm, cur.set[0]));
            if (two) MH_TRY(bbox_accumulate(c, d_mm, cur.set[1]));
            uint32_t mm[6];
            MH_TRY(read_back(c, mm, d_mm, sizeof mm));
            for (int d = 0; d < 3; ++d) {
                cur.lower[d] = ord2f(mm[d]) + (-cutoff - F32_EPS);
                cur.upper[d] = ord2f(mm[3 + d]) + (cutoff + F32_EPS);
            }
        }
        for (int d = 0; d < 3; ++d) ext[d] = cur.upper[d] - cur.lower[d];
    }
    MH_TRY(dims_from_extents(cur, ext));
    if (*reuse0 && !held_same_cells(c->held, cur)) {
        *reuse0 = false;
        c->held.valid = false;
        MH_TRY(stage_set(c, cur.set[0], q->xyz1, q->natoms1, q->idx1, q->n1, q->vdw1, vdw));
    }
    *to_hold = (may_hold && !*reuse0) ? held_remember(*q, cur, fp) : HeldGrid{};
    occ_latch(c);
    cur.ntasks = plan_entries(cur);
    cur.nslots_bound = slots_bound(cur, call.hist_plan);
    if (cur.ntasks >= 0xFFFFFFF0ull || cur.nslots_bound >= 0xFFFFFFF0ull || cur.ntasks + cur.nslots_bound >= 0xFFFFFF00ull)
        return fail(MOLAR_HIP_ERR_TOO_LARGE, "search plan too large (%llu entries)", (unsigned long long)cur.ntasks);
    return 0;
}

int reserve_plan(molar_hip_ctx *c, const SearchCall &call) {
    const SearchShape &cur = c->cur;
    MH_TRY(c->task_nb.reserve((cur.ntasks + 1) * 4));
    MH_TRY(c->task_desc.reserve((cur.ntasks + 1) * sizeof(TaskDesc)));
    MH_TRY(c->slot_desc.reserve((cur.nslots_bound + 1) * sizeof(SlotDesc)));
    if (call.hist_plan) MH_TRY(c->slot_desc_rest.reserve((cur.nslots_bound + 1) * sizeof(SlotDesc)));
    MH_TRY(c->slot_cnt.reserve((cur.nslots_bound + 1) * 4));
    MH_TRY(c->slot_base.reserve((cur.nslots_bound + 1) * 8));
    MH_TRY(c->params.reserve(sizeof(SearchParams)));
    MH_TRY(c->scan_state.reserve((lookback_state_words(cur.ntasks + 1) + lookback_state_words(cur.nslots_bound + 1)) * 8));
    MH_TRY(c->task_mu.reserve((cur.ntasks + 1) * 4));
    MH_TRY(c->task_moff.reserve((cur.ntasks + 1) * 8));
    MH_TRY(c->slot_stat.reserve(16));
    return 0;
}

bool plans_live_rows(const SearchCall &call, const SearchShape &cur) { return call.plan && call.live_rows && !call.hist_plan && live_row_slots(cur); }

int enqueue_live_rows(molar_hip_ctx *c, const SearchCall &call, const GridLane &lane) {
    const SearchShape &cur = c->cur;
    if (!plans_live_rows(call, cur)) return 0;
    MH_TRY(cur.set[0].live.reserve(live_rows_bytes(cur)));
    unsigned long long *masks = cur.set[0].live.as<unsigned long long>();
    uint32_t *cnt = reinterpret_cast<uint32_t *>(masks + live_rows_mask_words(cur));
    const SearchParams P = make_params(c, cur);
    const dim3 grid = pair_grid((unsigned)cur.ntasks);
    if (cur.kind == MOLAR_HIP_SEARCH_SINGLE) hipLaunchKernelGGL((live_rows_kernel<MOLAR_HIP_SEARCH_SINGLE>), grid, dim3(64), 0, lane.stream, P, masks, cnt);
    else hipLaunchKernelGGL((live_rows_kernel<MOLAR_HIP_SEARCH_DOUBLE>), grid, dim3(64), 0, lane.stream, P, masks, cnt);
    MH_HIP(hipGetLastError());
    return 0;
}

int build_grids(molar_hip_ctx *c, const SearchCall &call, const GridLane &lane, bool build0, int ids_local) {
    SearchShape &cur = c->cur;
    if (build0) MH_TRY(build_grid(c, call, lane, cur.set[0], ids_local));
    if (cur.kind != MOLAR_HIP_SEARCH_SINGLE) MH_TRY(build_grid(c, call, lane, cur.set[1], ids_local));
    return enqueue_live_rows(c, call, lane);
}

int enqueue_plan(molar_hip_ctx *c, const SearchCall &call) {
    Prof prof(c, 0);
    const SearchShape &cur = c->cur;
    const uint32_t fast_kind = records_hit_history(cur) ? 1u : 0u;
    const bool use_live = plans_live_rows(call, cur);
    SearchParams P = make_params(c, cur);
    SearchParams *params_dst = nullptr;
    c->params_fresh = false;
    if (!call.size_masks) {
        P.out_cap = call.out_cap;
        params_dst = c->params.as<SearchParams>();
        c->params_fresh = true;
        c->params_fresh_cap = P.out_cap;
    }
    if (cur.ntasks + 1 <= FPLAN_MAX_TASKS) {
        const uint32_t ntiles = (uint32_t)((cur.ntasks + 1 + 255) / 256);
        const uint32_t ngroups = ntiles > 1024u ? (ntiles + PLAN_GROUP - 1u) / PLAN_GROUP : 0u;
        MH_TRY(c->fplan_tiles.reserve((size_t)ntiles * 16 + (cur.ntasks + 1) * 8 + (size_t)ngroups * 16));
        unsigned long long *moff = fast_kind ? c->task_moff.as<unsigned long long>() : nullptr;
        unsigned long long *tt = c->fplan_tiles.as<unsigned long long>();
        unsigned long long *lmoff = tt + 2 * (size_t)ntiles;
        uint32_t *lfirst = c->task_mu.as<uint32_t>();
        const unsigned long long *live_masks = use_live ? cur.set[0].live.as<unsigned long long>() : nullptr;
        const uint32_t *live_cnt = use_live ? reinterpret_cast<const uint32_t *>(live_masks + live_rows_mask_words(cur)) : nullptr;
        if (cur.kind == MOLAR_HIP_SEARCH_SINGLE)
            hipLaunchKernelGGL((plan_tiles_kernel<MOLAR_HIP_SEARCH_SINGLE>), dim3(ntiles), dim3(256), 0, c->stream, P, lfirst,
                               c->task_desc.as<TaskDesc>(), lmoff, fast_kind, c->slot_cnt.as<uint32_t>(), cur.nslots_bound + 1, tt, params_dst, live_cnt);
        else
            hipLaunchKernelGGL((plan_tiles_kernel<MOLAR_HIP_SEARCH_DOUBLE>), dim3(ntiles), dim3(256), 0, c->stream, P, lfirst,
                               c->task_desc.as<TaskDesc>(), lmoff, fast_kind, c->slot_cnt.as<uint32_t>(), cur.nslots_bound + 1, tt, params_dst, live_cnt);
        unsigned long long *gt = ngroups ? lmoff + (cur.ntasks + 1) : nullptr;
// ... 81 lines not shown
        tot = sizes->total;
        occ_note(c, occ_key_of(c->cur), *sizes);
    } else {
        MH_TRY(read_back(c, &tot, c->slot_base.as<unsigned long long>() + c->cur.nslots_bound, 8));
    }
    c->total = tot;
    c->have_search = true;
    return 0;
}

}

extern "C" {

int molar_hip_search_count(molar_hip_ctx *c, const molar_hip_search_desc *q, uint64_t *out_count) {
    SearchCall call;
    bool degenerate;
    MH_TRY(prepare_search(c, q, call, &degenerate));
    if (degenerate) {
        c->have_search = true;
        if (out_count) *out_count = 0;
        return MOLAR_HIP_OK;
    }
    MH_TRY(launch_pairs<false>(c, call, PairOut{}));
    MH_TRY(finish_count(c));
    if (out_count) *out_count = c->total;
    return MOLAR_HIP_OK;
}

int molar_hip_search_grid_dims(molar_hip_ctx *c, uint64_t dims[3]) {
    if (!c || !c->have_search) return fail(MOLAR_HIP_ERR_NO_SEARCH, "no cached search: call molar_hip_search_count first");
    for (int d = 0; d < 3; ++d) dims[d] = c->cur.dims[d];
    return MOLAR_HIP_OK;
}

int molar_hip_search_cell_kernels(molar_hip_ctx *c, int32_t *lanes, uint64_t occupied_cells[2]) {
    if (!c || !lanes) return fail(MOLAR_HIP_ERR_INVALID_ARGUMENT, "search_cell_kernels: null argument");
    *lanes = pair_family(c->cur);
    if (occupied_cells) {
        occupied_cells[0] = c->cur.occ_use[0];
        occupied_cells[1] = c->cur.occ_use[1];
    }
    return MOLAR_HIP_OK;
}

int molar_hip_search_slot_counts(molar_hip_ctx *c, uint64_t *slots, uint64_t *consecutive_slots) {
    if (!c || !slots || !consecutive_slots) return fail(MOLAR_HIP_ERR_INVALID_ARGUMENT, "search_slot_counts: null argument");
    if (!c->slot_stat_valid) return fail(MOLAR_HIP_ERR_NO_SEARCH, "search_slot_counts: the context's last search was not planned by plan_slots_kernel");
    MH_HIP(hipSetDevice(c->device));
    unsigned long long st[2] = {0ull, 0ull};
    MH_TRY(read_back(c, st, c->slot_stat.p, sizeof st));
    *slots = st[0];
    *consecutive_slots = st[1];
    return MOLAR_HIP_OK;
}

static int fill_common(molar_hip_ctx *c, uint2 *d_pairs, float *d_dist, uint32_t *d_ids) {
    if (!c || !c->have_search) return fail(MOLAR_HIP_ERR_NO_SEARCH, "no cached search: call molar_hip_search_count first");
    MH_HIP(hipSetDevice(c->device));
    if (c->total == 0 || c->cur.ntasks == 0) return 0;
    uint2 *p = d_pairs;
    float *d = d_dist;
    const bool via_p = p && ((uintptr_t)p & 15u) != 0, via_d = d && ((uintptr_t)d & 7u) != 0;
    if (via_p) {
        MH_TRY(c->out_pairs.reserve((size_t)c->total * 8));
        p = c->out_pairs.as<uint2>();
    }
    if (via_d) {
        MH_TRY(c->out_dist.reserve((size_t)c->total * 4));
        d = c->out_dist.as<float>();
    }
    MH_TRY(launch_pairs<true>(c, SearchCall{}, PairOut{p, d, d_ids}));
    if (via_p) MH_HIP(hipMemcpyAsync(d_pairs, p, (size_t)c->total * 8, hipMemcpyDeviceToDevice, c->stream));
    if (via_d) MH_HIP(hipMemcpyAsync(d_dist, d, (size_t)c->total * 4, hipMemcpyDeviceToDevice, c->stream));
    return 0;
}

int molar_hip_search_fill(molar_hip_ctx *c, uint32_t *pairs, float *dist) {
    if (!c || !c->have_search) return fail(MOLAR_HIP_ERR_NO_SEARCH, "no cached search: call molar_hip_search_count first");
    if (c->cur.kind == MOLAR_HIP_SEARCH_WITHIN)
        return fail(MOLAR_HIP_ERR_INVALID_ARGUMENT, "within search yields ids: use molar_hip_search_fill_ids");
    const bool pd = is_device_ptr(pairs), dd = is_device_ptr(dist);
    uint2 *dp = nullptr;
    float *ddist = nullptr;
    if (pairs) {
        if (pd) dp = reinterpret_cast<uint2 *>(pairs);
        else {
            MH_TRY(c->out_pairs.reserve((size_t)(c->total ? c->total : 1) * 8));
            dp = c->out_pairs.as<uint2>();
        }
    }
    if (dist) {
        if (dd) ddist = dist;
        else {
            MH_TRY(c->out_dist.reserve((size_t)(c->total ? c->total : 1) * 4));
            ddist = c->out_dist.as<float>();
        }
    }
    MH_TRY(fill_common(c, dp, ddist, nullptr));
    const bool hp = pairs && !pd && c->total, hd = dist && !dd && c->total;
    if (ring_pays(c->total * ((hp ? 8u : 0u) + (hd ? 4u : 0u)), hp ? pairs : nullptr, hd ? dist : nullptr)) {
        std::vector<RingJob> jobs;
        if (hp) jobs.push_back(RingJob{dp, (size_t)c->total * 8, RING_COPY, pairs, nullptr});
        if (hd) jobs.push_back(RingJob{ddist, (size_t)c->total * 4, RING_COPY, dist, nullptr});
        return ring_to_host(c, jobs);
    }
// ... 628 lines not shown
```

molar_amd/csrc/search_shape.hpp:

```cpp
#pragma once

#include <algorithm>
#include <cmath>
#include <cstring>

#include "common.hpp"

namespace mh {

inline bool fixed_cutoff_kind(int kind) { return kind == MOLAR_HIP_SEARCH_SINGLE || kind == MOLAR_HIP_SEARCH_DOUBLE; }

inline uint64_t grid_cells(const SearchShape &s) { return (uint64_t)s.dims[0] * s.dims[1] * s.dims[2]; }

inline int dims_from_extents(SearchShape &s, const float ext[3]) {
    double cells = 1.0;
    for (int d = 0; d < 3; ++d) {
        const float q = std::floor(ext[d] / s.cutoff);
        uint64_t n = (q > 0.0f) ? (q >= 4.0e9f ? 4000000000ull : (uint64_t)q) : 0ull;
        if (n < 1) n = 1;
        s.dims[d] = (uint32_t)n;
        cells *= (double)n;
    }
    if (cells > 1.0e8)
        return fail(MOLAR_HIP_ERR_TOO_LARGE, "search grid %u x %u x %u has too many cells (cutoff %g)", s.dims[0],
// ... 9 lines not shown
inline int small_cell_lanes(const SearchShape &s) {
#ifdef MH_NO_SMALL_CELLS
    return 0;
#endif
    if (!fixed_cutoff_kind(s.kind)) return 0;
    int lanes = 16;
    const int nsets = s.kind == MOLAR_HIP_SEARCH_SINGLE ? 1 : 2;
    for (int k = 0; k < nsets; ++k) {
        const uint64_t cells = judged_cells(s, k), n = s.set[k].n;
        const int l = n <= 13ull * cells ? 16 : (n <= 19ull * cells ? 32 : 0);
        lanes = (l == 0 || lanes == 0) ? 0 : std::max(lanes, l);
    }
    return lanes;
}

inline int pair_family(const SearchShape &s) {
    if (const int lanes = small_cell_lanes(s)) return lanes;
    if (!fixed_cutoff_kind(s.kind)) return 0;
    const int b = s.kind == MOLAR_HIP_SEARCH_SINGLE ? 0 : 1;
    const uint64_t cells = judged_cells(s, b), n = s.set[b].n;
    return n > 1000ull * cells ? -2 : (n > 448ull * cells ? -1 : 0);
}

inline bool records_hit_history(const SearchShape &s) { return fixed_cutoff_kind(s.kind) && small_cell_lanes(s) == 0; }

inline bool sorted_by_device_sort(uint64_t n, uint64_t ncells) { return n > 384ull * ncells; }

inline unsigned long long occ_key_of(const SearchShape &s) {
    unsigned long long h = 1469598103934665603ull;
    auto mix = [&](unsigned long long v) { h = (h ^ v) * 1099511628211ull; };
    mix((unsigned long long)s.kind + 1u); mix(s.set[0].n); mix(s.kind == MOLAR_HIP_SEARCH_SINGLE ? 0u : s.set[1].n);
    mix(s.dims[0]); mix(s.dims[1]); mix(s.dims[2]); mix(s.use_box ? 1u : 2u);
    return h ? h : 1ull;
}

inline uint64_t plan_entries(const SearchShape &s) { return grid_cells(s) * 14ull * (s.kind != MOLAR_HIP_SEARCH_SINGLE ? 2ull : 1ull); }

inline uint64_t slots_bound(const SearchShape &s, bool hist_plan) {
    const uint64_t n0 = s.set[0].n;
    uint64_t bound = (s.kind != MOLAR_HIP_SEARCH_SINGLE ? 28ull : 14ull) * ((n0 + 63ull) / 64ull) + plan_entries(s) + 28ull * 512ull;
    if (hist_plan) bound += (n0 + 31ull) / 32ull + grid_cells(s);
    return bound;
}

constexpr uint64_t FPLAN_MAX_TASKS = 1ull << 22;

constexpr uint32_t LIVE_ROW_GROUPS = 8;
inline bool live_row_slots(const SearchShape &s) {
    return fixed_cutoff_kind(s.kind) && pair_family(s) == 0 && plan_entries(s) + 1 <= FPLAN_MAX_TASKS &&
           (plan_entries(s) <= 8192ull || (uint64_t)s.set[0].n >= 96ull * grid_cells(s));
}
inline size_t live_rows_mask_words(const SearchShape &s) { return (size_t)plan_entries(s) * LIVE_ROW_GROUPS; }
inline size_t live_rows_bytes(const SearchShape &s) { return live_rows_mask_words(s) * 8u + (size_t)plan_entries(s) * 4u; }

inline uint64_t held_fingerprint(const float *xyz, size_t natoms) {
    uint64_t fp = 0xcbf29ce484222325ull;
    auto mix = [&](size_t atom) {
        uint32_t w[3];
        std::memcpy(w, xyz + 3 * atom, 12);
        for (int k = 0; k < 3; ++k) fp = (fp ^ w[k]) * 0x100000001b3ull;
    };
    const size_t n = natoms, step = n > 512 ? n / 512 : 1;
    for (size_t a = 0; a < n && a < 64; ++a) mix(a);
    for (size_t a = 0; a < n; a += step) mix(a);
    for (size_t a = n > 64 ? n - 64 : 0; a < n; ++a) mix(a);
    return fp | 1ull;
}

inline bool held_names_request(const HeldGrid &h, const molar_hip_search_desc &q, const SearchShape &s, uint64_t fp) {
    return h.valid && h.fp == fp && h.set == s.set && h.xyz == q.xyz1 && h.natoms == q.natoms1 && h.idx == q.idx1 && h.n == q.n1 &&
           h.ids_local == q.ids_local && h.use_box == s.use_box && h.pbc == s.pbc &&
           (!s.use_box || std::memcmp(&h.box, &s.box, sizeof s.box) == 0);
}

inline bool held_same_cells(const HeldGrid &h, const SearchShape &s) {
    bool same = h.dims[0] == s.dims[0] && h.dims[1] == s.dims[1] && h.dims[2] == s.dims[2];
    for (int d = 0; d < 3 && !s.use_box; ++d) same = same && h.lower[d] == s.lower[d] && h.upper[d] == s.upper[d];
    return same;
}

inline HeldGrid held_remember(const molar_hip_search_desc &q, const SearchShape &s, uint64_t fp) {
    HeldGrid h;
    h.valid = true;
    h.set = s.set;
    h.fp = fp;
    h.xyz = q.xyz1; h.idx = q.idx1; h.natoms = q.natoms1; h.n = q.n1;
    h.ids_local = q.ids_local;
    h.use_box = s.use_box; h.pbc = s.pbc; h.box = s.box;
    for (int d = 0; d < 3; ++d) { h.dims[d] = s.dims[d]; h.lower[d] = s.lower[d]; h.upper[d] = s.upper[d]; }
    return h;
}

struct WrapPolicy {
    uint32_t wrap_kind;
    uint32_t prune_wrapped;
    uint32_t approx_wrapped;
    float band_lo, band_hi;
    float prune_limit2;
};

inline WrapPolicy wrapped_pair_policy(const SearchShape &s) {
    WrapPolicy W{};
    const float cutoff2 = s.cutoff * s.cutoff;
    W.wrap_kind = 3u;
    if (s.use_box) {
        const float *m = s.box.m, *iv = s.box.inv;
// ... 63 lines not shown
```

rust/molar_hip/src/ffi.rs:

```rust
#![allow(non_camel_case_types, clippy::too_many_arguments, clippy::missing_safety_doc)]

use std::os::raw::{c_char, c_int, c_void};

use crate::types::{
    MolarHipBox, MolarHipContactGroups, MolarHipCtx, MolarHipDensityGrid, MolarHipFitStream, MolarHipIntcoordSpec, MolarHipMembraneDesc, MolarHipMembraneOut, MolarHipMembranePatches, MolarHipMembranePlan, MolarHipMembraneState,
    MolarHipMembraneStateF64, MolarHipTcfSpec,
    MolarHipMembraneView, MolarHipSearchDesc, MolarHipSearchDescF64, MolarHipXtc,
};

pub struct MolarHipFns {
    pub create: unsafe extern "C" fn(c_int) -> *mut MolarHipCtx,
    pub destroy: unsafe extern "C" fn(*mut MolarHipCtx),
    pub last_error: unsafe extern "C" fn() -> *const c_char,
    pub version: unsafe extern "C" fn() -> *const c_char,
    pub device_count: unsafe extern "C" fn() -> c_int,
    pub set_stream: unsafe extern "C" fn(*mut MolarHipCtx, *mut c_void) -> c_int,
    pub synchronize: unsafe extern "C" fn(*mut MolarHipCtx) -> c_int,
    pub profile_enable: unsafe extern "C" fn(*mut MolarHipCtx, c_int) -> c_int,
    pub profile_read: unsafe extern "C" fn(*mut MolarHipCtx, *mut f32, *mut u64) -> c_int,
    pub copy_bandwidth: unsafe extern "C" fn(*mut MolarHipCtx, usize, c_int, *mut f32) -> c_int,
    pub write_bandwidth: unsafe extern "C" fn(*mut MolarHipCtx, usize, c_int, *mut f32) -> c_int,
    pub box_from_matrix: unsafe extern "C" fn(*const f32, *mut MolarHipBox) -> c_int,
    pub box_from_vectors_angles: unsafe extern "C" fn(f32, f32, f32, f32, f32, f32, *mut MolarHipBox) -> c_int,
    pub box_shortest_vector: unsafe extern "C" fn(*const MolarHipBox, *const f32, u8, *mut f32),
    pub box_lab_extents: unsafe extern "C" fn(*const MolarHipBox, *mut f32),
    pub box_extents: unsafe extern "C" fn(*const MolarHipBox, *mut f32),
    pub box_to_box_coords: unsafe extern "C" fn(*const MolarHipBox, *const f32, *mut f32),
    pub box_to_lab_coords: unsafe extern "C" fn(*const MolarHipBox, *const f32, *mut f32),
    pub box_is_inside: unsafe extern "C" fn(*const MolarHipBox, *const f32) -> c_int,
    pub box_wrap_point: unsafe extern "C" fn(*const MolarHipBox, *const f32, *mut f32),
    pub search_count: unsafe extern "C" fn(*mut MolarHipCtx, *const MolarHipSearchDesc, *mut u64) -> c_int,
    pub search_fill: unsafe extern "C" fn(*mut MolarHipCtx, *mut u32, *mut f32) -> c_int,
    pub search_fill_usize: unsafe extern "C" fn(*mut MolarHipCtx, *mut u64, *mut u64, *mut f32) -> c_int,
    pub search_fill_ids: unsafe extern "C" fn(*mut MolarHipCtx, *mut u64) -> c_int,
    pub within_count: unsafe extern "C" fn(*mut MolarHipCtx, *const MolarHipSearchDesc, *mut u64) -> c_int,
    pub within_fill: unsafe extern "C" fn(*mut MolarHipCtx, *mut u64) -> c_int,
    pub within_hold: unsafe extern "C" fn(*mut MolarHipCtx, c_int) -> c_int,
    pub search_connectivity: unsafe extern "C" fn(*mut MolarHipCtx, *const MolarHipSearchDesc, *mut u64, *mut u64) -> c_int,
    pub search_connectivity_fill: unsafe extern "C" fn(*mut MolarHipCtx, *mut u64, *mut u64) -> c_int,
    pub unwrap_connectivity: unsafe extern "C" fn(*mut MolarHipCtx, *mut f32, usize, *const u64, usize, *const f32, f32, u8, *mut u64, *mut u64, *mut usize) -> c_int,
    pub search_grid_dims: unsafe extern "C" fn(*mut MolarHipCtx, *mut u64) -> c_int,
    pub search_cell_kernels: unsafe extern "C" fn(*mut MolarHipCtx, *mut i32, *mut u64) -> c_int,
    pub search_slot_counts: unsafe extern "C" fn(*mut MolarHipCtx, *mut u64, *mut u64) -> c_int,
    pub search_fill_device: unsafe extern "C" fn(*mut MolarHipCtx, *mut *const u32, *mut *const f32) -> c_int,
    pub search_resident: unsafe extern "C" fn(*mut MolarHipCtx, *const MolarHipSearchDesc, *mut u64, *mut *const u32, *mut *const f32) -> c_int,
    pub search_resident_planes: unsafe extern "C" fn(*mut MolarHipCtx, c_int) -> c_int,
    pub search_resident_begin: unsafe extern "C" fn(*mut MolarHipCtx, *const MolarHipSearchDesc, *mut i32) -> c_int,
    pub search_resident_end: unsafe extern "C" fn(*mut MolarHipCtx, i32, *mut u64, *mut *const u32, *mut *const f32) -> c_int,
    pub search_histogram: unsafe extern "C" fn(*mut MolarHipCtx, *const MolarHipSearchDesc, f32, f32, usize, *mut u64, *mut u64) -> c_int,
    pub search_histogram_frames: unsafe extern "C" fn(*mut MolarHipCtx, *const MolarHipSearchDesc, usize, usize, usize, *const f32, f32, f32, usize, *mut u64) -> c_int,
    pub histogram_edges: unsafe extern "C" fn(f32, f32, usize, *mut f32) -> c_int,
    pub search_contacts: unsafe extern "C" fn(*mut MolarHipCtx, *const MolarHipSearchDesc, *const MolarHipContactGroups, *mut u64, *mut u64, *mut u64, *mut u64) -> c_int,
    pub search_contacts_frames: unsafe extern "C" fn(*mut MolarHipCtx, *const MolarHipSearchDesc, *const MolarHipContactGroups, usize, usize, usize, *const f32, *mut u64, *mut u64, *mut u64, *mut u32) -> c_int,
    pub search_clusters: unsafe extern "C" fn(*mut MolarHipCtx, *const MolarHipSearchDesc, *const MolarHipContactGroups, *mut u32, *mut u32, *mut u64, *mut u32, *mut u32) -> c_int,
    pub search_clusters_frames: unsafe extern "C" fn(*mut MolarHipCtx, *const MolarHipSearchDesc, *const MolarHipContactGroups, usize, usize, *const f32, *mut u32, *mut u32, *mut u64, *mut u32) -> c_int,
    pub search_clusters_counters: unsafe extern "C" fn(*mut MolarHipCtx, i32, *mut u64) -> c_int,
    pub hbonds_count: unsafe extern "C" fn(*mut MolarHipCtx, *const MolarHipSearchDesc, *const u64, *const u64, usize, i32, f64, f64, *mut u64) -> c_int,
    pub hbonds_fill: unsafe extern "C" fn(*mut MolarHipCtx, *mut u32, *mut f64, *mut f64, *mut f64) -> c_int,
    pub hbonds_counts: unsafe extern "C" fn(*mut MolarHipCtx, *const MolarHipSearchDesc, *const u64, *const u64, usize, i32, f64, f64, *const MolarHipContactGroups, *mut u64, *mut u64, *mut u64, *mut u64) -> c_int,
    pub hbonds_frames: unsafe extern "C" fn(*mut MolarHipCtx, *const MolarHipSearchDesc, *const u64, *const u64, usize, i32, f64, f64, usize, usize, *const f32, *const MolarHipContactGroups, *mut u64, *mut u64, *mut u64, *mut u64, *mut u64, *mut u64) -> c_int,
    pub hbonds_frames_fill: unsafe extern "C" fn(*mut MolarHipCtx, *mut u64, *mut u32, *mut f64, *mut f64, *mut f64, *mut u32, *mut u32, *mut u32) -> c_int,
    pub lifetimes_plan: unsafe extern "C" fn(usize, usize, usize, c_int, *mut usize, *mut u32) -> c_int,
    pub lifetimes: unsafe extern "C" fn(*mut MolarHipCtx, *const u64, *const u32, usize, usize, *const u32, usize, usize, usize, usize, *mut u64, *mut u64, *mut u64, *mut u32, *mut u32, *mut u32) -> c_int,
    pub hbonds_frames_shape: unsafe extern "C" fn(*mut MolarHipCtx, *mut usize, *mut usize, *mut usize, *mut u64) -> c_int,
    pub hbonds_frames_lifetimes: unsafe extern "C" fn(*mut MolarHipCtx, *const u32, usize, usize, usize, usize, *mut u64, *mut u64, *mut u64, *mut u32, *mut u32, *mut u32) -> c_int,
    pub search_count_f64: unsafe extern "C" fn(*mut MolarHipCtx, *const MolarHipSearchDescF64, *mut u64) -> c_int,
    pub search_fill_f64: unsafe extern "C" fn(*mut MolarHipCtx, *mut u64, *mut u64, *mut f64) -> c_int,
    pub search_fill_ids_f64: unsafe extern "C" fn(*mut MolarHipCtx, *mut u64) -> c_int,
    pub search_grid_dims_f64: unsafe extern "C" fn(*mut MolarHipCtx, *mut u64) -> c_int,
    pub search_histogram_f64: unsafe extern "C" fn(*mut MolarHipCtx, *const MolarHipSearchDescF64, f64, f64, usize, *mut u64, *mut u64) -> c_int,
    pub search_histogram_frames_f64: unsafe extern "C" fn(*mut MolarHipCtx, *const MolarHipSearchDescF64, usize, usize, usize, *const f64, f64, f64, usize, *mut u64) -> c_int,
    pub histogram_edges_f64: unsafe extern "C" fn(f64, f64, usize, *mut f64) -> c_int,
    pub within_count_f64: unsafe extern "C" fn(*mut MolarHipCtx, *const MolarHipSearchDescF64, *mut u64) -> c_int,
    pub within_fill_f64: unsafe extern "C" fn(*mut MolarHipCtx, *mut u64) -> c_int,
    pub search_connectivity_f64: unsafe extern "C" fn(*mut MolarHipCtx, *const MolarHipSearchDescF64, *mut u64, *mut u64) -> c_int,
    pub unwrap_connectivity_f64: unsafe extern "C" fn(*mut MolarHipCtx, *mut f64, usize, *const u64, usize, *const f64, f64, u8, *mut u64, *mut u64, *mut usize) -> c_int,
    pub min_max: unsafe extern "C" fn(*mut MolarHipCtx, *const f32, usize, *const u64, usize, *mut f32, *mut f32) -> c_int,
    pub center_of_geometry: unsafe extern "C" fn(*mut MolarHipCtx, *const f32, usize, *const u64, usize, *mut f32) -> c_int,
    pub center_of_mass: unsafe extern "C" fn(*mut MolarHipCtx, *const f32, usize, *const u64, usize, *const f32, *mut f32) -> c_int,
    pub center_of_geometry_pbc: unsafe extern "C" fn(*mut MolarHipCtx, *const f32, usize, *const u64, usize, *const f32, u8, *mut f32) -> c_int,
    pub center_of_mass_pbc: unsafe extern "C" fn(*mut MolarHipCtx, *const f32, usize, *const u64, usize, *const f32, *const f32, u8, *mut f32) -> c_int,
    pub gyration: unsafe extern "C" fn(*mut MolarHipCtx, *const f32, usize, *const u64, usize, *const f32, *const f32, *mut f32) -> c_int,
    pub inertia: unsafe extern "C" fn(*mut MolarHipCtx, *const f32, usize, *const u64, usize, *const f32, *const f32, *mut f32, *mut f32, *mut f32) -> c_int,
    pub rmsd: unsafe extern "C" fn(*mut MolarHipCtx, *const f32, usize, *const u64, usize, *const f32, usize, *const u64, usize, *mut f32) -> c_int,
    pub rmsd_mw: unsafe extern "C" fn(*mut MolarHipCtx, *const f32, usize, *const u64, usize, *const f32, *const f32, usize, *const u64, usize, *mut f32) -> c_int,
    pub fit_transform: unsafe extern "C" fn(*mut MolarHipCtx, *const f32, usize, *const u64, usize, *const f32, *const f32, usize, *const u64, usize, *const f32, c_int, *mut f32, *mut f32) -> c_int,
    pub center_of_geometry_f64: unsafe extern "C" fn(*mut MolarHipCtx, *const f64, usize, *const u64, usize, *mut f64) -> c_int,
    pub center_of_mass_f64: unsafe extern "C" fn(*mut MolarHipCtx, *const f64, usize, *const u64, usize, *const f64, *mut f64) -> c_int,
    pub gyration_f64: unsafe extern "C" fn(*mut MolarHipCtx, *const f64, usize, *const u64, usize, *const f64, *mut f64) -> c_int,
    pub rmsd_f64: unsafe extern "C" fn(*mut MolarHipCtx, *const f64, usize, *const u64, usize, *const f64, usize, *const u64, usize, *mut f64) -> c_int,
    pub rmsd_mw_f64: unsafe extern "C" fn(*mut MolarHipCtx, *const f64, usize, *const u64, usize, *const f64, *const f64, usize, *const u64, usize, *mut f64) -> c_int,
    pub fit_transform_f64: unsafe extern "C" fn(*mut MolarHipCtx, *const f64, usize, *const u64, usize, *const f64, *const f64, usize, *const u64, usize, *const f64, c_int, *mut f64, *mut f64) -> c_int,
    pub min_max_f64: unsafe extern "C" fn(*mut MolarHipCtx, *const f64, usize, *const u64, usize, *mut f64, *mut f64) -> c_int,
    pub inertia_f64: unsafe extern "C" fn(*mut MolarHipCtx, *const f64, usize, *const u64, usize, *const f64, *mut f64, *mut f64, *mut f64) -> c_int,
    pub translate_f64: unsafe extern "C" fn(*mut MolarHipCtx, *mut f64, usize, *const u64, usize, *const f64) -> c_int,
    pub sasa_points: unsafe extern "C" fn(u32, *mut f32) -> c_int,
// ... 73 lines not shown
    pub xtc_encode_frame: unsafe extern "C" fn(*const f32, usize, *const f32, i32, f32, f32, *mut u8, usize, *mut usize) -> c_int,
    pub apply_transform: unsafe extern "C" fn(*mut MolarHipCtx, *mut f32, usize, *const u64, usize, *const f32, *const f32) -> c_int,
    pub unwrap_simple: unsafe extern "C" fn(*mut MolarHipCtx, *mut f32, usize, *const u64, usize, *const f32, u8) -> c_int,
    pub fit_rmsd_batch: unsafe extern "C" fn(*mut MolarHipCtx, *mut f32, usize, usize, *const u64, usize, *const f32, *const f32, usize, *const u64, c_int, *mut f32, *mut f32, *mut f32, *mut f32, *mut f32) -> c_int,
    pub fit_stream_create: unsafe extern "C" fn(*mut MolarHipCtx, usize, *const u64, usize, *const f32, *const f32, usize, *const u64, c_int, *mut *mut MolarHipFitStream) -> c_int,
    pub fit_stream_begin: unsafe extern "C" fn(*mut MolarHipFitStream, *mut f32, c_int, *mut i32) -> c_int,
    pub fit_stream_end: unsafe extern "C" fn(*mut MolarHipFitStream, i32, *mut f32, *mut f32, *mut f32, *mut f32, *mut f32) -> c_int,
    pub fit_stream_destroy: unsafe extern "C" fn(*mut MolarHipFitStream),
    pub gyration_batch: unsafe extern "C" fn(*mut MolarHipCtx, *const f32, usize, *const u64, *const u64, usize, *const f32, *const f32, *mut f32) -> c_int,
    pub rmsd_batch: unsafe extern "C" fn(*mut MolarHipCtx, *const f32, usize, *const u64, *const f32, usize, *const u64, *const u64, usize, *const f32, *mut f32) -> c_int,
    pub fit_batch: unsafe extern "C" fn(*mut MolarHipCtx, *mut f32, usize, *const u64, *const f32, *const f32, usize, *const u64, *const f32, *const u64, usize, c_int, *mut f32, *mut f32, *mut f32, *mut f32, *mut f32) -> c_int,
    pub translate: unsafe extern "C" fn(*mut MolarHipCtx, *mut f32, usize, *const u64, usize, *const f32) -> c_int,
    pub rotate: unsafe extern "C" fn(*mut MolarHipCtx, *mut f32, usize, *const u64, usize, *const f32, f32) -> c_int,
    pub principal_transform: unsafe extern "C" fn(*mut MolarHipCtx, *const f32, usize, *const u64, usize, *const f32, *const f32, *mut f32, *mut f32) -> c_int,
}

impl MolarHipFns {
    pub unsafe fn resolve(lib: &libloading::Library) -> Result<Self, libloading::Error> {
        unsafe {
            Ok(MolarHipFns {
                create: *lib.get::<unsafe extern "C" fn(c_int) -> *mut MolarHipCtx>(b"molar_hip_create\0")?,
                destroy: *lib.get::<unsafe extern "C" fn(*mut MolarHipCtx)>(b"molar_hip_destroy\0")?,
                last_error: *lib.get::<unsafe extern "C" fn() -> *const c_char>(b"molar_hip_last_error\0")?,
                version: *lib.get::<unsafe extern "C" fn() -> *const c_char>(b"molar_hip_version\0")?,
                device_count: *lib.get::<unsafe extern "C" fn() -> c_int>(b"molar_hip_device_count\0")?,
                set_stream: *lib.get::<unsafe extern "C" fn(*mut MolarHipCtx, *mut c_void) -> c_int>(b"molar_hip_set_stream\0")?,
                synchronize: *lib.get::<unsafe extern "C" fn(*mut MolarHipCtx) -> c_int>(b"molar_hip_synchronize\0")?,
                profile_enable: *lib.get::<unsafe extern "C" fn(*mut MolarHipCtx, c_int) -> c_int>(b"molar_hip_profile_enable\0")?,
                profile_read: *lib.get::<unsafe extern "C" fn(*mut MolarHipCtx, *mut f32, *mut u64) -> c_int>(b"molar_hip_profile_read\0")?,
                copy_bandwidth: *lib.get::<unsafe extern "C" fn(*mut MolarHipCtx, usize, c_int, *mut f32) -> c_int>(b"molar_hip_copy_bandwidth\0")?,
                write_bandwidth: *lib.get::<unsafe extern "C" fn(*mut MolarHipCtx, usize, c_int, *mut f32) -> c_int>(b"molar_hip_write_bandwidth\0")?,
                box_from_matrix: *lib.get::<unsafe extern "C" fn(*const f32, *mut MolarHipBox) -> c_int>(b"molar_hip_box_from_matrix\0")?,
                box_from_vectors_angles: *lib.get::<unsafe extern "C" fn(f32, f32, f32, f32, f32, f32, *mut MolarHipBox) -> c_int>(b"molar_hip_box_from_vectors_angles\0")?,
                box_shortest_vector: *lib.get::<unsafe extern "C" fn(*const MolarHipBox, *const f32, u8, *mut f32)>(b"molar_hip_box_shortest_vector\0")?,
                box_lab_extents: *lib.get::<unsafe extern "C" fn(*const MolarHipBox, *mut f32)>(b"molar_hip_box_lab_extents\0")?,
                box_extents: *lib.get::<unsafe extern "C" fn(*const MolarHipBox, *mut f32)>(b"molar_hip_box_extents\0")?,
                box_to_box_coords: *lib.get::<unsafe extern "C" fn(*const MolarHipBox, *const f32, *mut f32)>(b"molar_hip_box_to_box_coords\0")?,
                box_to_lab_coords: *lib.get::<unsafe extern "C" fn(*const MolarHipBox, *const f32, *mut f32)>(b"molar_hip_box_to_lab_coords\0")?,
                box_is_inside: *lib.get::<unsafe extern "C" fn(*const MolarHipBox, *const f32) -> c_int>(b"molar_hip_box_is_inside\0")?,
                box_wrap_point: *lib.get::<unsafe extern "C" fn(*const MolarHipBox, *const f32, *mut f32)>(b"molar_hip_box_wrap_point\0")?,
                search_count: *lib.get::<unsafe extern "C" fn(*mut MolarHipCtx, *const MolarHipSearchDesc, *mut u64) -> c_int>(b"molar_hip_search_count\0")?,
                search_fill: *lib.get::<unsafe extern "C" fn(*mut MolarHipCtx, *mut u32, *mut f32) -> c_int>(b"molar_hip_search_fill\0")?,
                search_fill_usize: *lib.get::<unsafe extern "C" fn(*mut MolarHipCtx, *mut u64, *mut u64, *mut f32) -> c_int>(b"molar_hip_search_fill_usize\0")?,
                search_fill_ids: *lib.get::<unsafe extern "C" fn(*mut MolarHipCtx, *mut u64) -> c_int>(b"molar_hip_search_fill_ids\0")?,
                within_count: *lib.get::<unsafe extern "C" fn(*mut MolarHipCtx, *const MolarHipSearchDesc, *mut u64) -> c_int>(b"molar_hip_within_count\0")?,
                within_fill: *lib.get::<unsafe extern "C" fn(*mut MolarHipCtx, *mut u64) -> c_int>(b"molar_hip_within_fill\0")?,
                within_hold: *lib.get::<unsafe extern "C" fn(*mut MolarHipCtx, c_int) -> c_int>(b"molar_hip_within_hold\0")?,
                search_connectivity: *lib.get::<unsafe extern "C" fn(*mut MolarHipCtx, *const MolarHipSearchDesc, *mut u64, *mut u64) -> c_int>(b"molar_hip_search_connectivity\0")?,
                search_connectivity_fill: *lib.get::<unsafe extern "C" fn(*mut MolarHipCtx, *mut u64, *mut u64) -> c_int>(b"molar_hip_search_connectivity_fill\0")?,
                unwrap_connectivity: *lib.get::<unsafe extern "C" fn(*mut MolarHipCtx, *mut f32, usize, *const u64, usize, *const f32, f32, u8, *mut u64, *mut u64, *mut usize) -> c_int>(b"molar_hip_unwrap_connectivity\0")?,
                search_grid_dims: *lib.get::<unsafe extern "C" fn(*mut MolarHipCtx, *mut u64) -> c_int>(b"molar_hip_search_grid_dims\0")?,
                search_cell_kernels: *lib.get::<unsafe extern "C" fn(*mut MolarHipCtx, *mut i32, *mut u64) -> c_int>(b"molar_hip_search_cell_kernels\0")?,
                search_slot_counts: *lib.get::<unsafe extern "C" fn(*mut MolarHipCtx, *mut u64, *mut u64) -> c_int>(b"molar_hip_search_slot_counts\0")?,
                search_fill_device: *lib.get::<unsafe extern "C" fn(*mut MolarHipCtx, *mut *const u32, *mut *const f32) -> c_int>(b"molar_hip_search_fill_device\0")?,
                search_resident: *lib.get::<unsafe extern "C" fn(*mut MolarHipCtx, *const MolarHipSearchDesc, *mut u64, *mut *const u32, *mut *const f32) -> c_int>(b"molar_hip_search_resident\0")?,
                search_resident_planes: *lib.get::<unsafe extern "C" fn(*mut MolarHipCtx, c_int) -> c_int>(b"molar_hip_search_resident_planes\0")?,
                search_resident_begin: *lib.get::<unsafe extern "C" fn(*mut MolarHipCtx, *const MolarHipSearchDesc, *mut i32) -> c_int>(b"molar_hip_search_resident_begin\0")?,
                search_resident_end: *lib.get::<unsafe extern "C" fn(*mut MolarHipCtx, i32, *mut u64, *mut *const u32, *mut *const f32) -> c_int>(b"molar_hip_search_resident_end\0")?,
                search_histogram: *lib.get::<unsafe extern "C" fn(*mut MolarHipCtx, *const MolarHipSearchDesc, f32, f32, usize, *mut u64, *mut u64) -> c_int>(b"molar_hip_search_histogram\0")?,
                search_histogram_frames: *lib.get::<unsafe extern "C" fn(*mut MolarHipCtx, *const MolarHipSearchDesc, usize, usize, usize, *const f32, f32, f32, usize, *mut u64) -> c_int>(b"molar_hip_search_histogram_frames\0")?,
                histogram_edges: *lib.get::<unsafe extern "C" fn(f32, f32, usize, *mut f32) -> c_int>(b"molar_hip_histogram_edges\0")?,
                search_contacts: *lib.get::<unsafe extern "C" fn(*mut MolarHipCtx, *const MolarHipSearchDesc, *const MolarHipContactGroups, *mut u64, *mut u64, *mut u64, *mut u64) -> c_int>(b"molar_hip_search_contacts\0")?,
                search_contacts_frames: *lib.get::<unsafe extern "C" fn(*mut MolarHipCtx, *const MolarHipSearchDesc, *const MolarHipContactGroups, usize, usize, usize, *const f32, *mut u64, *mut u64, *mut u64, *mut u32) -> c_int>(b"molar_hip_search_contacts_frames\0")?,
                search_clusters: *lib.get::<unsafe extern "C" fn(*mut MolarHipCtx, *const MolarHipSearchDesc, *const MolarHipContactGroups, *mut u32, *mut u32, *mut u64, *mut u32, *mut u32) -> c_int>(b"molar_hip_search_clusters\0")?,
                search_clusters_frames: *lib.get::<unsafe extern "C" fn(*mut MolarHipCtx, *const MolarHipSearchDesc, *const MolarHipContactGroups, usize, usize, *const f32, *mut u32, *mut u32, *mut u64, *mut u32) -> c_int>(b"molar_hip_search_clusters_frames\0")?,
                search_clusters_counters: *lib.get::<unsafe extern "C" fn(*mut MolarHipCtx, i32, *mut u64) -> c_int>(b"molar_hip_search_clusters_counters\0")?,
                hbonds_count: *lib.get::<unsafe extern "C" fn(*mut MolarHipCtx, *const MolarHipSearchDesc, *const u64, *const u64, usize, i32, f64, f64, *mut u64) -> c_int>(b"molar_hip_hbonds_count\0")?,
                hbonds_fill: *lib.get::<unsafe extern "C" fn(*mut MolarHipCtx, *mut u32, *mut f64, *mut f64, *mut f64) -> c_int>(b"molar_hip_hbonds_fill\0")?,
                hbonds_counts: *lib.get::<unsafe extern "C" fn(*mut MolarHipCtx, *const MolarHipSearchDesc, *const u64, *const u64, usize, i32, f64, f64, *const MolarHipContactGroups, *mut u64, *mut u64, *mut u64, *mut u64) -> c_int>(b"molar_hip_hbonds_counts\0")?,
                hbonds_frames: *lib.get::<unsafe extern "C" fn(*mut MolarHipCtx, *const MolarHipSearchDesc, *const u64, *const u64, usize, i32, f64, f64, usize, usize, *const f32, *const MolarHipContactGroups, *mut u64, *mut u64, *mut u64, *mut u64, *mut u64, *mut u64) -> c_int>(b"molar_hip_hbonds_frames\0")?,
                hbonds_frames_fill: *lib.get::<unsafe extern "C" fn(*mut MolarHipCtx, *mut u64, *mut u32, *mut f64, *mut f64, *mut f64, *mut u32, *mut u32, *mut u32) -> c_int>(b"molar_hip_hbonds_frames_fill\0")?,
                lifetimes_plan: *lib.get::<unsafe extern "C" fn(usize, usize, usize, c_int, *mut usize, *mut u32) -> c_int>(b"molar_hip_lifetimes_plan\0")?,
                lifetimes: *lib.get::<unsafe extern "C" fn(*mut MolarHipCtx, *const u64, *const u32, usize, usize, *const u32, usize, usize, usize, usize, *mut u64, *mut u64, *mut u64, *mut u32, *mut u32, *mut u32) -> c_int>(b"molar_hip_lifetimes\0")?,
                hbonds_frames_shape: *lib.get::<unsafe extern "C" fn(*mut MolarHipCtx, *mut usize, *mut usize, *mut usize, *mut u64) -> c_int>(b"molar_hip_hbonds_frames_shape\0")?,
                hbonds_frames_lifetimes: *lib.get::<unsafe extern "C" fn(*mut MolarHipCtx, *const u32, usize, usize, usize, usize, *mut u64, *mut u64, *mut u64, *mut u32, *mut u32, *mut u32) -> c_int>(b"molar_hip_hbonds_frames_lifetimes\0")?,
                search_count_f64: *lib.get::<unsafe extern "C" fn(*mut MolarHipCtx, *const MolarHipSearchDescF64, *mut u64) -> c_int>(b"molar_hip_search_count_f64\0")?,
                search_fill_f64: *lib.get::<unsafe extern "C" fn(*mut MolarHipCtx, *mut u64, *mut u64, *mut f64) -> c_int>(b"molar_hip_search_fill_f64\0")?,
                search_fill_ids_f64: *lib.get::<unsafe extern "C" fn(*mut MolarHipCtx, *mut u64) -> c_int>(b"molar_hip_search_fill_ids_f64\0")?,
                search_grid_dims_f64: *lib.get::<unsafe extern "C" fn(*mut MolarHipCtx, *mut u64) -> c_int>(b"molar_hip_search_grid_dims_f64\0")?,
                search_histogram_f64: *lib.get::<unsafe extern "C" fn(*mut MolarHipCtx, *const MolarHipSearchDescF64, f64, f64, usize, *mut u64, *mut u64) -> c_int>(b"molar_hip_search_histogram_f64\0")?,
                search_histogram_frames_f64: *lib.get::<unsafe extern "C" fn(*mut MolarHipCtx, *const MolarHipSearchDescF64, usize, usize, usize, *const f64, f64, f64, usize, *mut u64) -> c_int>(b"molar_hip_search_histogram_frames_f64\0")?,
                histogram_edges_f64: *lib.get::<unsafe extern "C" fn(f64, f64, usize, *mut f64) -> c_int>(b"molar_hip_histogram_edges_f64\0")?,
                within_count_f64: *lib.get::<unsafe extern "C" fn(*mut MolarHipCtx, *const MolarHipSearchDescF64, *mut u64) -> c_int>(b"molar_hip_within_count_f64\0")?,
                within_fill_f64: *lib.get::<unsafe extern "C" fn(*mut MolarHipCtx, *mut u64) -> c_int>(b"molar_hip_within_fill_f64\0")?,
                search_connectivity_f64: *lib.get::<unsafe extern "C" fn(*mut MolarHipCtx, *const MolarHipSearchDescF64, *mut u64, *mut u64) -> c_int>(b"molar_hip_search_connectivity_f64\0")?,
                unwrap_connectivity_f64: *lib.get::<unsafe extern "C" fn(*mut MolarHipCtx, *mut f64, usize, *const u64, usize, *const f64, f64, u8, *mut u64, *mut u64, *mut usize) -> c_int>(b"molar_hip_unwrap_connectivity_f64\0")?,
                min_max: *lib.get::<unsafe extern "C" fn(*mut MolarHipCtx, *const f32, usize, *const u64, usize, *mut f32, *mut f32) -> c_int>(b"molar_hip_min_max\0")?,
                center_of_geometry: *lib.get::<unsafe extern "C" fn(*mut MolarHipCtx, *const f32, usize, *const u64, usize, *mut f32) -> c_int>(b"molar_hip_center_of_geometry\0")?,
                center_of_mass: *lib.get::<unsafe extern "C" fn(*mut MolarHipCtx, *const f32, usize, *const u64, usize, *const f32, *mut f32) -> c_int>(b"molar_hip_center_of_mass\0")?,
                center_of_geometry_pbc: *lib.get::<unsafe extern "C" fn(*mut MolarHipCtx, *const f32, usize, *const u64, usize, *const f32, u8, *mut f32) -> c_int>(b"molar_hip_center_of_geometry_pbc\0")?,
                center_of_mass_pbc: *lib.get::<unsafe extern "C" fn(*mut MolarHipCtx, *const f32, usize, *const u64, usize, *const f32, *const f32, u8, *mut f32) -> c_int>(b"molar_hip_center_of_mass_pbc\0")?,
                gyration: *lib.get::<unsafe extern "C" fn(*mut MolarHipCtx, *const f32, usize, *const u64, usize, *const f32, *const f32, *mut f32) -> c_int>(b"molar_hip_gyration\0")?,
                inertia: *lib.get::<unsafe extern "C" fn(*mut MolarHipCtx, *const f32, usize, *const u64, usize, *const f32, *const f32, *mut f32, *mut f32, *mut f32) -> c_int>(b"molar_hip_inertia\0")?,
                rmsd: *lib.get::<unsafe extern "C" fn(*mut MolarHipCtx, *const f32, usize, *const u64, usize, *const f32, usize, *const u64, usize, *mut f32) -> c_int>(b"molar_hip_rmsd\0")?,
                rmsd_mw: *lib.get::<unsafe extern "C" fn(*mut MolarHipCtx, *const f32, usize, *const u64, usize, *const f32, *const f32, usize, *const u64, usize, *mut f32) -> c_int>(b"molar_hip_rmsd_mw\0")?,
                fit_transform: *lib.get::<unsafe extern "C" fn(*mut MolarHipCtx, *const f32, usize, *const u64, usize, *const f32, *const f32, usize, *const u64, usize, *const f32, c_int, *mut f32, *mut f32) -> c_int>(b"molar_hip_fit_transform\0")?,
                center_of_geometry_f64: *lib.get::<unsafe extern "C" fn(*mut MolarHipCtx, *const f64, usize, *const u64, usize, *mut f64) -> c_int>(b"molar_hip_center_of_geometry_f64\0")?,
                center_of_mass_f64: *lib.get::<unsafe extern "C" fn(*mut MolarHipCtx, *const f64, usize, *const u64, usize, *const f64, *mut f64) -> c_int>(b"molar_hip_center_of_mass_f64\0")?,
                gyration_f64: *lib.get::<unsafe extern "C" fn(*mut MolarHipCtx, *const f64, usize, *const u64, usize, *const f64, *mut f64) -> c_int>(b"molar_hip_gyration_f64\0")?,
                rmsd_f64: *lib.get::<unsafe extern "C" fn(*mut MolarHipCtx, *const f64, usize, *const u64, usize, *const f64, usize, *const u64, usize, *mut f64) -> c_int>(b"molar_hip_rmsd_f64\0")?,
                rmsd_mw_f64: *lib.get::<unsafe extern "C" fn(*mut MolarHipCtx, *const f64, usize, *const u64, usize, *const f64, *const f64, usize, *const u64, usize, *mut f64) -> c_int>(b"molar_hip_rmsd_mw_f64\0")?,
                fit_transform_f64: *lib.get::<unsafe extern "C" fn(*mut MolarHipCtx, *const f64, usize, *const u64, usize, *const f64, *const f64, usize, *const u64, usize, *const f64, c_int, *mut f64, *mut f64) -> c_int>(b"molar_hip_fit_transform_f64\0")?,
                min_max_f64: *lib.get::<unsafe extern "C" fn(*mut MolarHipCtx, *const f64, usize, *const u64, usize, *mut f64, *mut f64) -> c_int>(b"molar_hip_min_max_f64\0")?,
                inertia_f64: *lib.get::<unsafe extern "C" fn(*mut MolarHipCtx, *const f64, usize, *const u64, usize, *const f64, *mut f64, *mut f64, *mut f64) -> c_int>(b"molar_hip_inertia_f64\0")?,
                translate_f64: *lib.get::<unsafe extern "C" fn(*mut MolarHipCtx, *mut f64, usize, *const u64, usize, *const f64) -> c_int>(b"molar_hip_translate_f64\0")?,
                sasa_points: *lib.get::<unsafe extern "C" fn(u32, *mut f32) -> c_int>(b"molar_hip_sasa_points\0")?,
// ... 39 lines not shown
                inertia_pbc_f64: *lib.get::<unsafe extern "C" fn(*mut MolarHipCtx, *const f64, usize, *const u64, usize, *const f64, *const f64, *mut f64, *mut f64, *mut f64) -> c_int>(b"molar_hip_inertia_pbc_f64\0")?,
                apply_transform_f64: *lib.get::<unsafe extern "C" fn(*mut MolarHipCtx, *mut f64, usize, *const u64, usize, *const f64, *const f64) -> c_int>(b"molar_hip_apply_transform_f64\0")?,
                center_batch: *lib.get::<unsafe extern "C" fn(*mut MolarHipCtx, *const f32, usize, *const u64, *const u64, usize, *const f32, *mut f32) -> c_int>(b"molar_hip_center_batch\0")?,
                unwrap_simple_batch: *lib.get::<unsafe extern "C" fn(*mut MolarHipCtx, *mut f32, usize, *const u64, *const u64, usize, *const f32, u8) -> c_int>(b"molar_hip_unwrap_simple_batch\0")?,
                center_batch_f64: *lib.get::<unsafe extern "C" fn(*mut MolarHipCtx, *const f64, usize, *const u64, *const u64, usize, *const f64, *mut f64) -> c_int>(b"molar_hip_center_batch_f64\0")?,
                unwrap_simple_batch_f64: *lib.get::<unsafe extern "C" fn(*mut MolarHipCtx, *mut f64, usize, *const u64, *const u64, usize, *const f64, u8) -> c_int>(b"molar_hip_unwrap_simple_batch_f64\0")?,
                membrane_initial_normals: *lib.get::<unsafe extern "C" fn(usize, *const f32, *const f32, *const u64, *const u64, *const u8, *mut f32) -> c_int>(b"molar_hip_membrane_initial_normals\0")?,
                membrane_patches_from_pairs: *lib.get::<unsafe extern "C" fn(*const u32, usize, usize, *mut u64, *mut u64) -> c_int>(b"molar_hip_membrane_patches_from_pairs\0")?,
                membrane_smooth: *lib.get::<unsafe extern "C" fn(*mut MolarHipCtx, *const MolarHipMembranePatches, *const f32, *mut MolarHipMembraneState) -> c_int>(b"molar_hip_membrane_smooth\0")?,
                membrane_nth_shell_patches: *lib.get::<unsafe extern "C" fn(usize, *const u8, *const u64, *const u64, *const u32, *const u64, usize, *mut u64, *mut u64, usize, *mut usize) -> c_int>(b"molar_hip_membrane_nth_shell_patches\0")?,
                membrane_smooth_curvature: *lib.get::<unsafe extern "C" fn(usize, *const u8, *const u64, *const u32, *const u64, usize, *mut f32, *mut f32) -> c_int>(b"molar_hip_membrane_smooth_curvature\0")?,
                membrane_smooth_f64: *lib.get::<unsafe extern "C" fn(*mut MolarHipCtx, *const MolarHipMembranePatches, *const f64, *mut MolarHipMembraneStateF64) -> c_int>(b"molar_hip_membrane_smooth_f64\0")?,
                membrane_initial_normals_f64: *lib.get::<unsafe extern "C" fn(usize, *const f64, *const f64, *const u64, *const u64, *const u8, *mut f64) -> c_int>(b"molar_hip_membrane_initial_normals_f64\0")?,
                membrane_smooth_curvature_f64: *lib.get::<unsafe extern "C" fn(usize, *const u8, *const u64, *const u32, *const u64, usize, *mut f64, *mut f64) -> c_int>(b"molar_hip_membrane_smooth_curvature_f64\0")?,
                membrane_plan_create: *lib.get::<unsafe extern "C" fn(*mut MolarHipCtx, *const MolarHipMembraneDesc, *mut *mut MolarHipMembranePlan) -> c_int>(b"molar_hip_membrane_plan_create\0")?,
                membrane_plan_destroy: *lib.get::<unsafe extern "C" fn(*mut MolarHipMembranePlan)>(b"molar_hip_membrane_plan_destroy\0")?,
                membrane_plan_set_valid: *lib.get::<unsafe extern "C" fn(*mut MolarHipMembranePlan, *const u8) -> c_int>(b"molar_hip_membrane_plan_set_valid\0")?,
                membrane_plan_set_shells: *lib.get::<unsafe extern "C" fn(*mut MolarHipMembranePlan, usize, usize) -> c_int>(b"molar_hip_membrane_plan_set_shells\0")?,
                membrane_frame_begin: *lib.get::<unsafe extern "C" fn(*mut MolarHipMembranePlan, *mut f32, *const f32, *mut i32) -> c_int>(b"molar_hip_membrane_frame_begin\0")?,
                membrane_frame_end: *lib.get::<unsafe extern "C" fn(*mut MolarHipMembranePlan, i32, *mut MolarHipMembraneView) -> c_int>(b"molar_hip_membrane_frame_end\0")?,
                membrane_frame_fetch: *lib.get::<unsafe extern "C" fn(*mut MolarHipMembranePlan, i32, *const MolarHipMembraneOut) -> c_int>(b"molar_hip_membrane_frame_fetch\0")?,
                membrane_frame_end_fetch: *lib.get::<unsafe extern "C" fn(*mut MolarHipMembranePlan, i32, *mut MolarHipMembraneView, *const MolarHipMembraneOut) -> c_int>(b"molar_hip_membrane_frame_end_fetch\0")?,
                lipid_tail_order: *lib.get::<unsafe extern "C" fn(*mut MolarHipCtx, *const f32, usize, *const u64, *const u64, usize, c_int, *const f32, *const u64, *const u8, *mut f32) -> c_int>(b"molar_hip_lipid_tail_order\0")?,
                xtc_open: *lib.get::<unsafe extern "C" fn(*const c_char) -> *mut MolarHipXtc>(b"molar_hip_xtc_open\0")?,
                xtc_open_memory: *lib.get::<unsafe extern "C" fn(*const c_void, usize) -> *mut MolarHipXtc>(b"molar_hip_xtc_open_memory\0")?,
                xtc_close: *lib.get::<unsafe extern "C" fn(*mut MolarHipXtc)>(b"molar_hip_xtc_close\0")?,
                xtc_nframes: *lib.get::<unsafe extern "C" fn(*const MolarHipXtc) -> usize>(b"molar_hip_xtc_nframes\0")?,
                xtc_natoms: *lib.get::<unsafe extern "C" fn(*const MolarHipXtc) -> usize>(b"molar_hip_xtc_natoms\0")?,
                xtc_frame_info: *lib.get::<unsafe extern "C" fn(*const MolarHipXtc, usize, *mut i32, *mut i32, *mut f32, *mut f32, *mut f32) -> c_int>(b"molar_hip_xtc_frame_info\0")?,
                xtc_seek_time: *lib.get::<unsafe extern "C" fn(*const MolarHipXtc, f32, *mut usize) -> c_int>(b"molar_hip_xtc_seek_time\0")?,
                xtc_read: *lib.get::<unsafe extern "C" fn(*mut MolarHipCtx, *const MolarHipXtc, usize, usize, *mut f32, c_int) -> c_int>(b"molar_hip_xtc_read\0")?,
                xtc_read_device: *lib.get::<unsafe extern "C" fn(*mut MolarHipCtx, *const MolarHipXtc, usize, usize, *mut f32) -> c_int>(b"molar_hip_xtc_read_device\0")?,
                xtc_histogram: *lib.get::<unsafe extern "C" fn(*mut MolarHipCtx, *const MolarHipXtc, usize, usize, *const u64, usize, f32, u8, f32, f32, usize, *mut u64, c_int) -> c_int>(b"molar_hip_xtc_histogram\0")?,
                xtc_histogram_double: *lib.get::<unsafe extern "C" fn(*mut MolarHipCtx, *const MolarHipXtc, usize, usize, *const u64, usize, *const u64, usize, f32, u8, f32, f32, usize, *mut u64, c_int) -> c_int>(b"molar_hip_xtc_histogram_double\0")?,
                xtc_encode_frame: *lib.get::<unsafe extern "C" fn(*const f32, usize, *const f32, i32, f32, f32, *mut u8, usize, *mut usize) -> c_int>(b"molar_hip_xtc_encode_frame\0")?,
                apply_transform: *lib.get::<unsafe extern "C" fn(*mut MolarHipCtx, *mut f32, usize, *const u64, usize, *const f32, *const f32) -> c_int>(b"molar_hip_apply_transform\0")?,
                unwrap_simple: *lib.get::<unsafe extern "C" fn(*mut MolarHipCtx, *mut f32, usize, *const u64, usize, *const f32, u8) -> c_int>(b"molar_hip_unwrap_simple\0")?,
                fit_rmsd_batch: *lib.get::<unsafe extern "C" fn(*mut MolarHipCtx, *mut f32, usize, usize, *const u64, usize, *const f32, *const f32, usize, *const u64, c_int, *mut f32, *mut f32, *mut f32, *mut f32, *mut f32) -> c_int>(b"molar_hip_fit_rmsd_batch\0")?,
                fit_stream_create: *lib.get::<unsafe extern "C" fn(*mut MolarHipCtx, usize, *const u64, usize, *const f32, *const f32, usize, *const u64, c_int, *mut *mut MolarHipFitStream) -> c_int>(b"molar_hip_fit_stream_create\0")?,
                fit_stream_begin: *lib.get::<unsafe extern "C" fn(*mut MolarHipFitStream, *mut f32, c_int, *mut i32) -> c_int>(b"molar_hip_fit_stream_begin\0")?,
                fit_stream_end: *lib.get::<unsafe extern "C" fn(*mut MolarHipFitStream, i32, *mut f32, *mut f32, *mut f32, *mut f32, *mut f32) -> c_int>(b"molar_hip_fit_stream_end\0")?,
                fit_stream_destroy: *lib.get::<unsafe extern "C" fn(*mut MolarHipFitStream)>(b"molar_hip_fit_stream_destroy\0")?,
                gyration_batch: *lib.get::<unsafe extern "C" fn(*mut MolarHipCtx, *const f32, usize, *const u64, *const u64, usize, *const f32, *const f32, *mut f32) -> c_int>(b"molar_hip_gyration_batch\0")?,
                rmsd_batch: *lib.get::<unsafe extern "C" fn(*mut MolarHipCtx, *const f32, usize, *const u64, *const f32, usize, *const u64, *const u64, usize, *const f32, *mut f32) -> c_int>(b"molar_hip_rmsd_batch\0")?,
                fit_batch: *lib.get::<unsafe extern "C" fn(*mut MolarHipCtx, *mut f32, usize, *const u64, *const f32, *const f32, usize, *const u64, *const f32, *const u64, usize, c_int, *mut f32, *mut f32, *mut f32, *mut f32, *mut f32) -> c_int>(b"molar_hip_fit_batch\0")?,
                translate: *lib.get::<unsafe extern "C" fn(*mut MolarHipCtx, *mut f32, usize, *const u64, usize, *const f32) -> c_int>(b"molar_hip_translate\0")?,
                rotate: *lib.get::<unsafe extern "C" fn(*mut MolarHipCtx, *mut f32, usize, *const u64, usize, *const f32, f32) -> c_int>(b"molar_hip_rotate\0")?,
                principal_transform: *lib.get::<unsafe extern "C" fn(*mut MolarHipCtx, *const f32, usize, *const u64, usize, *const f32, *const f32, *mut f32, *mut f32) -> c_int>(b"molar_hip_principal_transform\0")?,
            })
        }
    }
}

pub const ENTRY_POINTS: usize = 173;
```

Before: 752.0 frames/s.

## Record per-row step hints in count pass to skip empty chunks in fill

During the MFMA count pass on live-row slots, each row gets a bitmask of which 64-atom neighbour chunks hold any candidate pair, reduced across lanes with DPP and written to a new per-slot hint buffer. The fill pass reads that byte for each row and skips distance evaluation for chunks marked empty. This is meant to avoid the redundant second sweep over chunks that produce no pairs. In exchange the count pass does extra DPP work and global writes, the fill pass does an extra load, and correctness depends on the hints staying consistent between the two passes. A diagnostic entry point reports hint statistics.

```diff
diff --git a/include/molar_hip.h b/include/molar_hip.h
--- a/include/molar_hip.h
+++ b/include/molar_hip.h
@@ -111,6 +111,7 @@
 int molar_hip_search_grid_dims(molar_hip_ctx *ctx, uint64_t dims[3]);
 int molar_hip_search_cell_kernels(molar_hip_ctx *ctx, int32_t *lanes, uint64_t occupied_cells[2]);
 int molar_hip_search_slot_counts(molar_hip_ctx *ctx, uint64_t *slots, uint64_t *consecutive_slots);
+int molar_hip_search_step_hints(molar_hip_ctx *ctx, uint64_t *slots, uint64_t *steps, uint64_t *clear_steps);
 int molar_hip_search_fill_device(molar_hip_ctx *ctx, const uint32_t **d_pairs, const float **d_dist);
 int molar_hip_search_resident(molar_hip_ctx *ctx, const molar_hip_search_desc *desc, uint64_t *out_count,
                               const uint32_t **d_pairs, const float **d_dist);
diff --git a/molar_amd/_lib.py b/molar_amd/_lib.py
--- a/molar_amd/_lib.py
+++ b/molar_amd/_lib.py
@@ -125,6 +125,7 @@
     "molar_hip_search_grid_dims": (_I, [_P, _P]),
     "molar_hip_search_cell_kernels": (_I, [_P, _P, _P]),
     "molar_hip_search_slot_counts": (_I, [_P, _P, _P]),
+    "molar_hip_search_step_hints": (_I, [_P, _P, _P, _P]),
     "molar_hip_search_count_f64": (_I, [_P, _P, _P]),
     "molar_hip_search_fill_f64": (_I, [_P, _P, _P, _P]),
     "molar_hip_search_fill_ids_f64": (_I, [_P, _P]),
diff --git a/molar_amd/api.py b/molar_amd/api.py
--- a/molar_amd/api.py
+++ b/molar_amd/api.py
@@ -278,6 +278,11 @@
         slots, rows = C.c_uint64(0), C.c_uint64(0)
         check(self.lib.molar_hip_search_slot_counts(self.ctx, C.byref(slots), C.byref(rows)))
         return int(slots.value), int(rows.value)
+
+    def search_step_hints(self):
+        slots, steps, clear = C.c_uint64(0), C.c_uint64(0), C.c_uint64(0)
+        check(self.lib.molar_hip_search_step_hints(self.ctx, C.byref(slots), C.byref(steps), C.byref(clear)))
+        return int(slots.value), int(steps.value), int(clear.value)
 
     def search_resident_planes(self, want_dist=True):
         check(self.lib.molar_hip_search_resident_planes(self.ctx, 1 if want_dist else 0))
diff --git a/molar_amd/csrc/api.hip b/molar_amd/csrc/api.hip
--- a/molar_amd/csrc/api.hip
+++ b/molar_amd/csrc/api.hip
@@ -153,6 +153,7 @@
     c->env_host_grid_wait = std::getenv("MOLAR_HIP_HOST_GRID_WAIT") != nullptr;
     c->env_no_bin_tile = std::getenv("MOLAR_HIP_NO_BIN_TILE") != nullptr;
 #endif
+    c->env_no_step_hints = std::getenv("MOLAR_HIP_NO_STEP_HINTS") != nullptr;
 #ifdef MOLAR_HIP_DEBUG_KNOBS
     if (const char *dbg = std::getenv("MOLAR_HIP_DEBUG_SKIP")) c->env_debug_skip = (uint32_t)std::atoi(dbg);
     if (const char *dbg = std::getenv("MOLAR_HIP_DEBUG_LAUNCH")) c->env_debug_launch = (uint32_t)std::atoi(dbg);
diff --git a/molar_amd/csrc/common.hpp b/molar_amd/csrc/common.hpp
--- a/molar_amd/csrc/common.hpp
+++ b/molar_amd/csrc/common.hpp
@@ -227,6 +227,7 @@
     uint32_t env_debug_skip = 0;
     uint32_t env_debug_launch = 0, dbg_launches = 0;
     hipEvent_t gen_free[2] = {nullptr, nullptr};
+    bool env_no_step_hints = false;
     bool env_no_bin_tile = false;
     int hist_gen = 0;
     mh::DevBuf scan_tmp_side;
@@ -292,6 +293,7 @@
     mh::DevBuf task_mu;
     mh::DevBuf task_moff;
     mh::DevBuf maskbuf;
+    mh::DevBuf hintbuf;
     uint64_t mask_units = 0;
 
     molar_hip_ctx *aux = nullptr;
diff --git a/molar_amd/csrc/pair_kernels.hpp b/molar_amd/csrc/pair_kernels.hpp
--- a/molar_amd/csrc/pair_kernels.hpp
+++ b/molar_amd/csrc/pair_kernels.hpp
@@ -101,6 +101,8 @@
     molar_hip_box box;
     alignas(16) float shifts4[96];
     uint32_t hist_big;
+    uint8_t *hints;
+    unsigned long long hint_cap_slots;
 };
 
 struct TaskDesc {
@@ -128,7 +130,13 @@
 struct SlotTask : Task {
     bool live = false;
     uint32_t lrow = 0;
+    uint32_t hslot = 0;
 };
+
+constexpr uint32_t STEP_HINT_BYTES = 64;
+__device__ __forceinline__ uint8_t *slot_hints(const SearchParams &P, const SlotTask &T) {
+    return (T.live && P.hints && T.hslot < P.hint_cap_slots) ? P.hints + (size_t)T.hslot * STEP_HINT_BYTES : nullptr;
+}
 
 __device__ __forceinline__ uint32_t slot_row(const SlotTask &T, uint32_t i0, uint32_t lane) { return T.live ? T.lrow : i0 + lane; }
 
@@ -753,6 +761,9 @@
     lds_u32 *todo = (lds_u32 *)lh;
     uint32_t ntodo = 0;
     uint32_t cnt = 0;
+    uint8_t *hints = nullptr;
+    if constexpr (!TRI) hints = slot_hints(P, T);
+    uint32_t hq[2] = {0u, 0u}, hbytes = 0u;
 #pragma unroll
     for (int t = 0; t < MFMA_TILES; ++t) {
         if ((uint32_t)t < nct) {
@@ -787,9 +798,32 @@
                 } else {
                     if (lane == 0) todo[ntodo] = (uint32_t)(2 * t + rt);
                     ++ntodo;
-                }
-            }
-        }
+                    h = 0xFFFFu;
+                }
+                if (!TRI && hints) hq[rt] |= h << (16 * ((t >> 1) & 1));
+            }
+            if (!TRI && hints && ((t & 3) == 3 || (uint32_t)t + 1u == nct)) {
+#pragma unroll
+                for (int rt = 0; rt < 2; ++rt) {
+                    if (32u * (uint32_t)rt >= nlive) continue;
+                    uint32_t x = hq[rt];
+                    x |= (uint32_t)__builtin_amdgcn_update_dpp(0, (int)x, 0xB1, 0xF, 0xF, false);
+                    x |= (uint32_t)__builtin_amdgcn_update_dpp(0, (int)x, 0x4E, 0xF, 0xF, false);
+                    x |= (uint32_t)__builtin_amdgcn_update_dpp(0, (int)x, 0x141, 0xF, 0xF, false);
+                    x |= (uint32_t)__builtin_amdgcn_update_dpp(0, (int)x, 0x140, 0xF, 0xF, false);
+                    x |= (uint32_t)__builtin_amdgcn_update_dpp(0, (int)x, 0x142, 0xA, 0xF, false);
+                    hbytes |= ((x >> (15u - (cl & 15u))) & 0x00010001u) << (2 * (t >> 2) + 8 * rt);
+                    hq[rt] = 0u;
+                }
+            }
+        }
+    }
+    if (!TRI && hints && cl >= 16u) {
+        const uint32_t i = cl & 15u, row = 8u * (i >> 2) + 4u * kh + (i & 3u);
+        typedef __attribute__((address_space(1))) uint8_t glb_u8;
+        hbytes = (hbytes & 0x5555u) | ((hbytes >> 15) & 0xAAAAu);
+        ((glb_u8 *)hints)[row] = (uint8_t)hbytes;
+        if (nlive > 32u) ((glb_u8 *)hints)[32u + row] = (uint8_t)(hbytes >> 8);
     }
     if (ntodo) {
         __builtin_amdgcn_wave_barrier();
@@ -990,6 +1024,15 @@
         }
     }
     constexpr bool REPLAY = FILL && MASKED;
+    constexpr bool HINTED = FILL && !WRAPPED && !TRI && !MASKED;
+    uint32_t hbyte = 0xFFu;
+    bool hinted = false;
+    if constexpr (HINTED) {
+        if (const uint8_t *hints = slot_hints(P, T)) {
+            hinted = true;
+            hbyte = ((const __attribute__((address_space(1))) uint8_t *)hints)[lane];
+        }
+    }
     float bx[NCH], by[NCH], bz[NCH];
     uint32_t bid[NCH];
     if (!REPLAY) {
@@ -1120,8 +1163,10 @@
         const float4 p = lload4(la, r);
         const uint32_t id_i = __float_as_uint(p.w);
         const uint32_t i = i0 + r;
+        const uint32_t steps = (HINTED && hinted) ? (uint32_t)__builtin_amdgcn_readlane((int)hbyte, (int)r) : 0xFFu;
 #pragma unroll
         for (int k = 0; k < NCH; ++k) {
+            if (HINTED && k < 8 && !((steps >> k) & 1u)) continue;
             if (TRI && (uint32_t)k * 64u + 63u <= i) {
                 if (MASKED && !FILL) hw[k] += hw[k];
                 continue;
@@ -1280,6 +1325,12 @@
             const uint32_t cm = (KIND == MOLAR_HIP_SEARCH_SINGLE && T.tri) ? run_count_mfma<KIND, true>(P, T, i0, la, F.lh, lane, done)
                                                                           : run_count_mfma<KIND, false>(P, T, i0, la, F.lh, lane, done);
             if (done) return cm;
+        }
+        if (!T.tri) {
+            if (uint8_t *hints = slot_hints(P, T)) {
+                typedef __attribute__((address_space(1))) uint8_t glb_u8;
+                ((glb_u8 *)hints)[lane] = (uint8_t)0xFFu;
+            }
         }
     }
     if constexpr (!FILL && MASKED && WK != WK_NONE && (KIND == MOLAR_HIP_SEARCH_SINGLE || KIND == MOLAR_HIP_SEARCH_DOUBLE)) {
@@ -1495,6 +1546,7 @@
                     T.lrow = scr[lane];
                     __builtin_amdgcn_wave_barrier();
                     T.live = true;
+                    T.hslot = slot;
                     T.n1 = before;
                 }
             }
diff --git a/molar_amd/csrc/search.hip b/molar_amd/csrc/search.hip
--- a/molar_amd/csrc/search.hip
+++ b/molar_amd/csrc/search.hip
@@ -1086,6 +1086,28 @@
                                                         unsigned long long *__restrict__ out) {
     for (uint64_t k = (uint64_t)blockIdx.x * 256u + threadIdx.x; k < n; k += (uint64_t)gridDim.x * 256u)
         out[k] = ids[k];
+}
+
+__global__ void __launch_bounds__(64) step_hint_stat_kernel(const SlotDesc *__restrict__ slot_desc, uint32_t nslots, const uint8_t *__restrict__ hints,
+                                                            unsigned long long cap_slots, unsigned long long *__restrict__ out) {
+    const uint32_t slot = blockIdx.y * gridDim.x + blockIdx.x, lane = threadIdx.x;
+    if (slot >= nslots || slot >= cap_slots) return;
+    const SlotDesc S = slot_desc[slot];
+    const uint32_t fl = S.flags;
+    if (!(fl & 0x200u) || !(fl & SLOT_LIVE) || (fl & 0x100u) || (fl & 7u) || S.n2 > 64u * (uint32_t)KREG) return;
+    const unsigned long long *mk = reinterpret_cast<const unsigned long long *>(S.pad1);
+    uint32_t nl = lane < (uint32_t)LIVE_GROUPS ? (uint32_t)__popcll(mk[lane]) : 0u;
+    for (int off = 32; off > 0; off >>= 1) nl += __shfl_xor(nl, off, 64);
+    const uint32_t rows = nl > S.i0 ? (nl - S.i0 < 64u ? nl - S.i0 : 64u) : 0u;
+    const uint32_t nch = (S.n2 + 63u) >> 6;
+    uint32_t clear = 0u;
+    if (lane < rows) clear = nch - (uint32_t)__popc((uint32_t)hints[(size_t)slot * STEP_HINT_BYTES + lane] & ((1u << nch) - 1u));
+    for (int off = 32; off > 0; off >>= 1) clear += __shfl_xor(clear, off, 64);
+    if (lane == 0 && rows) {
+        atomicAdd(out, 1ull);
+        atomicAdd(out + 1, (unsigned long long)rows * nch);
+        atomicAdd(out + 2, (unsigned long long)clear);
+    }
 }
 
 __global__ void upload_params_kernel(SearchParams P, SearchParams *dst) {
@@ -1256,6 +1278,8 @@
     P.maskbuf = c->maskbuf.as<uint32_t>();
     P.task_moff = c->task_moff.as<unsigned long long>();
     P.mask_cap_units = c->maskbuf.cap / 256u;
+    P.hints = c->env_no_step_hints ? nullptr : c->hintbuf.as<uint8_t>();
+    P.hint_cap_slots = c->hintbuf.cap / STEP_HINT_RECORD;
     P.out_cap = ~0ull;
     P.dx = shape.dims[0];
     P.dy = shape.dims[1];
@@ -1575,6 +1599,8 @@
     return 0;
 }
 
+bool plans_live_rows(const SearchCall &call, const SearchShape &cur) { return call.plan && call.live_rows && !call.hist_plan && live_row_slots(cur); }
+
 int reserve_plan(molar_hip_ctx *c, const SearchCall &call) {
     const SearchShape &cur = c->cur;
     MH_TRY(c->task_nb.reserve((cur.ntasks + 1) * 4));
@@ -1587,11 +1613,10 @@
     MH_TRY(c->scan_state.reserve((lookback_state_words(cur.ntasks + 1) + lookback_state_words(cur.nslots_bound + 1)) * 8));
     MH_TRY(c->task_mu.reserve((cur.ntasks + 1) * 4));
     MH_TRY(c->task_moff.reserve((cur.ntasks + 1) * 8));
-    MH_TRY(c->slot_stat.reserve(16));
+    MH_TRY(c->slot_stat.reserve(40));
+    if (!c->env_no_step_hints && plans_live_rows(call, cur)) MH_TRY(c->hintbuf.reserve(step_hint_bytes(cur.nslots_bound)));
     return 0;
 }
-
-bool plans_live_rows(const SearchCall &call, const SearchShape &cur) { return call.plan && call.live_rows && !call.hist_plan && live_row_slots(cur); }
 
 int enqueue_live_rows(molar_hip_ctx *c, const SearchCall &call, const GridLane &lane) {
     const SearchShape &cur = c->cur;
@@ -1779,6 +1804,26 @@
     MH_TRY(read_back(c, st, c->slot_stat.p, sizeof st));
     *slots = st[0];
     *consecutive_slots = st[1];
+    return MOLAR_HIP_OK;
+}
+
+int molar_hip_search_step_hints(molar_hip_ctx *c, uint64_t *slots, uint64_t *steps, uint64_t *clear_steps) {
+    if (!c || !slots || !steps || !clear_steps) return fail(MOLAR_HIP_ERR_INVALID_ARGUMENT, "search_step_hints: null argument");
+    *slots = *steps = *clear_steps = 0;
+    if (!c->slot_stat_valid) return fail(MOLAR_HIP_ERR_NO_SEARCH, "search_step_hints: the context's last search was not planned by plan_slots_kernel");
+    if (!c->plan_live || c->env_no_step_hints || !c->hintbuf.p) return MOLAR_HIP_OK;
+    MH_HIP(hipSetDevice(c->device));
+    unsigned long long *d = c->slot_stat.as<unsigned long long>() + 2;
+    MH_HIP(hipMemsetAsync(d, 0, 24, c->stream));
+    const uint32_t n = (uint32_t)c->cur.nslots_bound;
+    hipLaunchKernelGGL(step_hint_stat_kernel, pair_grid(n), dim3(64), 0, c->stream, c->slot_desc.as<SlotDesc>(), n, c->hintbuf.as<uint8_t>(),
+                       (unsigned long long)(c->hintbuf.cap / STEP_HINT_RECORD), d);
+    MH_HIP(hipGetLastError());
+    unsigned long long st[3] = {0ull, 0ull, 0ull};
+    MH_TRY(read_back(c, st, d, sizeof st));
+    *slots = st[0];
+    *steps = st[1];
+    *clear_steps = st[2];
     return MOLAR_HIP_OK;
 }
 
diff --git a/molar_amd/csrc/search_shape.hpp b/molar_amd/csrc/search_shape.hpp
--- a/molar_amd/csrc/search_shape.hpp
+++ b/molar_amd/csrc/search_shape.hpp
@@ -85,6 +85,9 @@
 }
 inline size_t live_rows_mask_words(const SearchShape &s) { return (size_t)plan_entries(s) * LIVE_ROW_GROUPS; }
 inline size_t live_rows_bytes(const SearchShape &s) { return live_rows_mask_words(s) * 8u + (size_t)plan_entries(s) * 4u; }
+
+constexpr size_t STEP_HINT_RECORD = 64;
+inline size_t step_hint_bytes(uint64_t nslots_bound) { return (size_t)(nslots_bound + 1u) * STEP_HINT_RECORD; }
 
 inline uint64_t held_fingerprint(const float *xyz, size_t natoms) {
     uint64_t fp = 0xcbf29ce484222325ull;
diff --git a/rust/molar_hip/src/ffi.rs b/rust/molar_hip/src/ffi.rs
--- a/rust/molar_hip/src/ffi.rs
+++ b/rust/molar_hip/src/ffi.rs
@@ -42,6 +42,7 @@
     pub search_grid_dims: unsafe extern "C" fn(*mut MolarHipCtx, *mut u64) -> c_int,
     pub search_cell_kernels: unsafe extern "C" fn(*mut MolarHipCtx, *mut i32, *mut u64) -> c_int,
     pub search_slot_counts: unsafe extern "C" fn(*mut MolarHipCtx, *mut u64, *mut u64) -> c_int,
+    pub search_step_hints: unsafe extern "C" fn(*mut MolarHipCtx, *mut u64, *mut u64, *mut u64) -> c_int,
     pub search_fill_device: unsafe extern "C" fn(*mut MolarHipCtx, *mut *const u32, *mut *const f32) -> c_int,
     pub search_resident: unsafe extern "C" fn(*mut MolarHipCtx, *const MolarHipSearchDesc, *mut u64, *mut *const u32, *mut *const f32) -> c_int,
     pub search_resident_planes: unsafe extern "C" fn(*mut MolarHipCtx, c_int) -> c_int,
@@ -221,6 +222,7 @@
                 search_grid_dims: *lib.get::<unsafe extern "C" fn(*mut MolarHipCtx, *mut u64) -> c_int>(b"molar_hip_search_grid_dims\0")?,
                 search_cell_kernels: *lib.get::<unsafe extern "C" fn(*mut MolarHipCtx, *mut i32, *mut u64) -> c_int>(b"molar_hip_search_cell_kernels\0")?,
                 search_slot_counts: *lib.get::<unsafe extern "C" fn(*mut MolarHipCtx, *mut u64, *mut u64) -> c_int>(b"molar_hip_search_slot_counts\0")?,
+                search_step_hints: *lib.get::<unsafe extern "C" fn(*mut MolarHipCtx, *mut u64, *mut u64, *mut u64) -> c_int>(b"molar_hip_search_step_hints\0")?,
                 search_fill_device: *lib.get::<unsafe extern "C" fn(*mut MolarHipCtx, *mut *const u32, *mut *const f32) -> c_int>(b"molar_hip_search_fill_device\0")?,
                 search_resident: *lib.get::<unsafe extern "C" fn(*mut MolarHipCtx, *const MolarHipSearchDesc, *mut u64, *mut *const u32, *mut *const f32) -> c_int>(b"molar_hip_search_resident\0")?,
                 search_resident_planes: *lib.get::<unsafe extern "C" fn(*mut MolarHipCtx, c_int) -> c_int>(b"molar_hip_search_resident_planes\0")?,
@@ -366,4 +368,4 @@
     }
 }
 
-pub const ENTRY_POINTS: usize = 173;
+pub const ENTRY_POINTS: usize = 174;
```

Result: no change. 759.9 frames/s (median of 5 runs) (+1.1%).
